# CliMA/ClimaOcean.jl

Measured on AMD Instinct MI355X. Metric: flux-kernel surface cells/s (update_state!: JRA55 interp + similarity-theory fluxes + net fluxes), higher is better.
Workload: dtype f64; 1 GPU; 1/4-degree LatitudeLongitudeGrid surface 1440x560 per job, JRA55 640x320 f32 atmosphere (4-snapshot window, clock advancing 20 min per step), SimilarityTheoryFluxes(:default) + Radiation, halo 7, ring 1; global_cells=806400, parallelism=latitude-slab x1, rows_per_rank=560, halo_backend=none, halo_rows=0, pipelined_interpolation=True, pipeline_mode=tail, step_loop=cf_time_steps (C)

## Files before the change

climaocean.jl_amd/coflux/abi.py:

```python
import ctypes as C
import os

import numpy as np

ABI_VERSION = 5
COMM_ID_BYTES = 128
PEER_HANDLE_BYTES = 64
HALO_NONE, HALO_RCCL, HALO_PEER = 0, 1, 2
FOLD_CENTER, FOLD_X_FACE, FOLD_Y_FACE = 0, 1, 2
SKIN_EXPLICIT, SKIN_SEMI_IMPLICIT, SKIN_LINEARISED = 0, 1, 2

SIMILARITY_LOGARITHMIC, SIMILARITY_COARE_LOGARITHMIC = 0, 1
STABILITY_EDSON2013, STABILITY_SHEBA, STABILITY_LARGE_YEAGER = 0, 1, 2
ROUGHNESS_CONSTANT, ROUGHNESS_CHARNOCK, ROUGHNESS_WIND_CHARNOCK = 0, 1, 2
SCALAR_ROUGHNESS_CONSTANT, SCALAR_ROUGHNESS_REYNOLDS = 0, 1
VISCOSITY_CONSTANT, VISCOSITY_TEMPERATURE_DEPENDENT = 0, 1
STOP_CONVERGENCE, STOP_FIXED = 0, 1
FORMULATION_SIMILARITY, FORMULATION_LARGE_YEAGER = 0, 1
VELOCITY_RELATIVE, VELOCITY_WIND = 0, 1
MASK_NONE, MASK_U8, MASK_BOTTOM_HEIGHT = 0, 1, 2
ALBEDO_CONSTANT, ALBEDO_LATITUDE_DEPENDENT = 0, 1
OPT_SOLVER, OPT_TRIP_HINTS, OPT_FUSED_NET, OPT_ICE_ORBIT_SHORTCUT, OPT_MERGED_PREFETCH = 0, 3, 6, 7, 9
OPT_INTERP_TILE_CAP, OPT_AO_CHUNK = 1, 4
OPT_INTERP_TILE_ROWS = 15
OPT_SOLVER_PATH, OPT_CERTIFIED_BUDGET, OPT_ICE_FREE_CELLS, OPT_LATENCY_LAYOUT, OPT_HALO_IN_SOLVER_LAUNCH = 10, 11, 12, 13, 14
OPT_LAND_ZEROS = 2
LAND_ZEROS_EVERY_LAUNCH, LAND_ZEROS_AUTO, LAND_ZEROS_NEVER = 0, 1, 2
ICE_FREE_ITERATE, ICE_FREE_ZERO = 0, 1
PIPELINE_WITHIN_CALL, PIPELINE_CONTINUING = 1, 2
AVERAGE_MAX_FIELDS = 16
DERIVED_MAX_SOURCES = 16
(TERM_FIELD, TERM_PRODUCT, TERM_CENTER_X, TERM_CENTER_Y, TERM_CENTER_X_SQUARE, TERM_CENTER_Y_SQUARE, TERM_KINETIC_ENERGY,
 TERM_EAST, TERM_NORTH) = range(9)
TERM_AT_CENTERS = 1
(BUDGET_HEAT_SHORTWAVE, BUDGET_HEAT_LONGWAVE_UP, BUDGET_HEAT_LONGWAVE_DOWN, BUDGET_HEAT_SENSIBLE, BUDGET_HEAT_LATENT,
 BUDGET_HEAT_ATMOSPHERE_OCEAN, BUDGET_HEAT_ICE_OCEAN, BUDGET_HEAT_FRAZIL, BUDGET_HEAT_NET, BUDGET_SALT_EVAPORATION,
 BUDGET_SALT_PRECIPITATION, BUDGET_SALT_ATMOSPHERE_OCEAN, BUDGET_SALT_ICE_OCEAN, BUDGET_SALT_LAND,
 BUDGET_SALT_NET) = range(15)
BUDGET_KINDS = 15
ATTACHED_AVERAGES_MAX = 4
INTEGRALS_MAX_ENTRIES, INTEGRALS_MAX_FIELDS = 32, 32
INTEGRAND_ONE, INTEGRAND_FIELD, INTEGRAND_PRODUCT, INTEGRAND_ABOVE = 0, 1, 2, 3
MONITOR_MAX_ENTRIES = 16
MONITOR_VALUE, MONITOR_ABS = 0, 1
CLIMATOLOGY_MAX_FIELDS, CLIMATOLOGY_MAX_BINS = 16, 32
CHECKPOINT_MAX_SECTIONS = 256
CHECKPOINT_DIRECT = 1
REGRID_MAX_FIELDS = 16
REGRID_MEAN, REGRID_SUM = 0, 1
SOLVER_PATH_EXACT, SOLVER_PATH_CERTIFIED = 0, 1
CERTIFIED_EXACT_FLAG = 0x100
SOLVER_TABLES, SOLVER_LIBM = 0, 1
STAGE_INTERPOLATE, STAGE_AO_FLUXES, STAGE_NET_FLUXES, STAGE_UPDATE_STATE = 0, 1, 2, 3

JRA55_VARIABLES = ("tas", "huss", "psl", "uas", "vas", "rlds", "rsds", "prra", "prsn")
JRA55_NVARS = len(JRA55_VARIABLES)

c_double_p = C.POINTER(C.c_double)
c_float_p = C.POINTER(C.c_float)
c_int32_p = C.POINTER(C.c_int32)


class Grid(C.Structure):
    _fields_ = [("nx", C.c_int32), ("ny", C.c_int32), ("hx", C.c_int32), ("hy", C.c_int32),
                ("ring", C.c_int32), ("reserved", C.c_int32)]


class Roughness(C.Structure):
    _fields_ = [("kind", C.c_int32), ("viscosity_kind", C.c_int32),
                ("constant_length", C.c_double), ("maximum_length", C.c_double),
                ("charnock", C.c_double), ("laminar", C.c_double),
                ("wind_a1", C.c_double), ("wind_a2", C.c_double), ("wind_umax", C.c_double),
                ("reynolds_A", C.c_double), ("reynolds_b", C.c_double),
                ("viscosity", C.c_double * 4)]


class Thermodynamics(C.Structure):
    _fields_ = [("gas_constant", C.c_double), ("dry_air_molar_mass", C.c_double),
                ("water_molar_mass", C.c_double), ("kappa_d", C.c_double),
                ("cp_v", C.c_double), ("cp_l", C.c_double), ("cp_i", C.c_double),
                ("LH_v0", C.c_double), ("LH_s0", C.c_double),
                ("T_0", C.c_double), ("T_triple", C.c_double), ("p_triple", C.c_double),
                ("T_freeze", C.c_double), ("T_icenuc", C.c_double), ("pow_icenuc", C.c_double)]


class Seawater(C.Structure):
    _fields_ = [("water_molar_mass", C.c_double),
                ("constituent_molar_mass", C.c_double * 4),
                ("constituent_mass_fraction", C.c_double * 4)]


class FluxParams(C.Structure):
    _fields_ = [("struct_size", C.c_int32), ("abi_version", C.c_int32),
                ("similarity_form", C.c_int32), ("stability_functions", C.c_int32),
                ("stop_kind", C.c_int32), ("maxiter", C.c_int32),
                ("velocity_difference", C.c_int32), ("mask_kind", C.c_int32),
                ("tolerance", C.c_double), ("von_karman", C.c_double),
                ("gustiness_parameter", C.c_double), ("minimum_gustiness", C.c_double),
                ("shear_gustiness_coefficient", C.c_double),
                ("similarity_profile_floor", C.c_double),
                ("momentum_roughness", Roughness), ("temperature_roughness", Roughness),
                ("water_vapor_roughness", Roughness),
                ("reference_height", C.c_double), ("boundary_layer_height", C.c_double),
                ("gravitational_acceleration", C.c_double),
                ("thermo", Thermodynamics), ("seawater", Seawater),
                ("ocean_reference_density", C.c_double), ("ocean_heat_capacity", C.c_double),
                ("ocean_freshwater_density", C.c_double),
                ("ocean_temperature_offset", C.c_double), ("ocean_minimum_salinity", C.c_double),
                ("ocean_surface_z", C.c_double),
                ("ocean_albedo_kind", C.c_int32), ("penetrating_shortwave", C.c_int32),
# ... 136 lines not shown
class BudgetDesc(C.Structure):
    _fields_ = [("struct_size", C.c_int32), ("n_terms", C.c_int32), ("terms", C.POINTER(BudgetTerm)),
                ("ocean", C.POINTER(OceanSurface)), ("exchange", C.POINTER(ExchangeFields)), ("fluxes", C.POINTER(InterfaceFluxes)),
                ("ice", C.POINTER(SeaIceFields)), ("frazil_heat", C.c_void_p), ("land_freshwater", C.c_void_p),
                ("weights", C.POINTER(InterpWeights)), ("max_workgroups", C.c_int32), ("reserved", C.c_int32)]


class IntegralEntry(C.Structure):
    _fields_ = [("kind", C.c_int32), ("region_bit", C.c_int32), ("a", C.c_void_p), ("b", C.c_void_p),
                ("threshold", C.c_double)]


class IntegralsDesc(C.Structure):
    _fields_ = [("struct_size", C.c_int32), ("n_entries", C.c_int32),
                ("area", C.c_void_p), ("mask", C.c_void_p), ("region", C.c_void_p),
                ("max_workgroups", C.c_int32), ("reserved", C.c_int32),
                ("entries", IntegralEntry * INTEGRALS_MAX_ENTRIES)]


class MonitorEntry(C.Structure):
    _fields_ = [("a", C.c_void_p), ("kind", C.c_int32), ("reserved", C.c_int32)]


class MonitorDesc(C.Structure):
    _fields_ = [("struct_size", C.c_int32), ("n_entries", C.c_int32), ("mask", C.c_void_p), ("first_cell", C.c_int64),
                ("max_workgroups", C.c_int32), ("reserved", C.c_int32), ("entries", MonitorEntry * MONITOR_MAX_ENTRIES)]


class MonitorValue(C.Structure):
    _fields_ = [("minimum", C.c_double), ("maximum", C.c_double), ("argmin", C.c_int64), ("argmax", C.c_int64),
                ("nan_count", C.c_int64), ("inf_count", C.c_int64), ("first_nonfinite", C.c_int64), ("hash", C.c_uint64)]


MONITOR_VALUE_DTYPE = np.dtype([("minimum", "<f8"), ("maximum", "<f8"), ("argmin", "<i8"), ("argmax", "<i8"), ("nan_count", "<i8"),
                                ("inf_count", "<i8"), ("first_nonfinite", "<i8"), ("hash", "<u8")])
assert MONITOR_VALUE_DTYPE.itemsize == C.sizeof(MonitorValue) == 64


class ClimatologyDesc(C.Structure):
    _fields_ = [("struct_size", C.c_int32), ("n_fields", C.c_int32), ("n_bins", C.c_int32), ("max_workgroups", C.c_int32),
                ("sources", C.c_void_p * CLIMATOLOGY_MAX_FIELDS), ("totals", C.c_void_p * CLIMATOLOGY_MAX_FIELDS),
                ("bins", C.c_void_p * CLIMATOLOGY_MAX_FIELDS), ("reserved", C.c_int32 * 2)]


class DatasetDesc(C.Structure):
    _fields_ = [("struct_size", C.c_int32), ("ns_x", C.c_int32), ("ns_y", C.c_int32), ("n_levels", C.c_int32),
                ("periodic_x", C.c_int32), ("max_sweeps", C.c_int32), ("sweeps_per_launch", C.c_int32), ("max_workgroups", C.c_int32),
                ("fill_value", C.c_double), ("period", C.c_double), ("times", C.c_void_p), ("weights", InterpWeights)]


class RegridDesc(C.Structure):
    _fields_ = [("struct_size", C.c_int32), ("mode", C.c_int32), ("n_rows", C.c_int64), ("nnz", C.c_int64),
                ("row_ptr", C.c_void_p), ("col", C.c_void_p), ("weight", C.c_void_p), ("mask", C.c_void_p),
                ("max_workgroups", C.c_int32), ("reserved", C.c_int32)]


class CheckpointDesc(C.Structure):
    _fields_ = [("struct_size", C.c_int32), ("flags", C.c_int32), ("max_workgroups", C.c_int32), ("reserved", C.c_int32)]


class PrefetchStats(C.Structure):
    _fields_ = [("struct_size", C.c_int32), ("pending", C.c_int32)] + [(n, C.c_uint64) for n in (
        "requests", "launched_aux", "launched_tail", "launched_merged", "launched_ice_tail", "launched_own",
        "consumed", "mismatched", "voided", "superseded", "discarded", "step_interpolations")]


EXPORTED_SYMBOLS = (
    "cf_version", "cf_default_flux_params", "cf_create", "cf_destroy", "cf_last_error",
    "cf_set_flux_params", "cf_set_stream", "cf_set_option", "cf_debug_eval", "cf_debug_chunk_plan", "cf_sync",
    "cf_device_alloc", "cf_device_free", "cf_h2d", "cf_d2h",
    "cf_interpolate_atmosphere_state", "cf_compute_atmosphere_ocean_fluxes",
    "cf_compute_net_ocean_fluxes", "cf_update_state", "cf_normalize_salinity_flux",
    "cf_default_sea_ice_params", "cf_set_sea_ice_formulation", "cf_compute_atmosphere_sea_ice_fluxes",
    "cf_compute_net_sea_ice_fluxes", "cf_update_state_sea_ice",
    "cf_time_stage", "cf_time_copy", "cf_profile_enable", "cf_profile_read",
    "cf_comm_unique_id", "cf_comm_init", "cf_comm_destroy", "cf_halo_exchange_rows",
    "cf_peer_halo_export", "cf_peer_halo_connect", "cf_halo_exchange_rows_peer", "cf_peer_halo_stats", "cf_fold_north_halo",
    "cf_time_steps", "cf_prefetch_atmosphere_state",
    "cf_default_sea_ice_albedo_params", "cf_set_sea_ice_albedo", "cf_compute_sea_ice_albedo",
    "cf_default_ice_ocean_params", "cf_compute_sea_ice_ocean_fluxes",
    "cf_interpolate_land_freshwater", "cf_set_land_freshwater", "cf_materialize_salinity_restoring",
    "cf_window_create", "cf_window_destroy", "cf_window_host_buffer", "cf_window_wait_slot", "cf_window_commit",
    "cf_window_upload", "cf_window_find", "cf_window_source",
    "cf_ensure_chunk_table", "cf_debug_chunk_table", "cf_debug_interp_grid", "cf_debug_land_zero_launches", "cf_solver_path", "cf_solver_iteration_path", "cf_solver_latency_layout", "cf_comm_count", "cf_build_stamp", "cf_discard_prefetched_atmosphere_state",
    "cf_debug_prefetch_stats",
    "cf_average_create", "cf_average_destroy", "cf_average_reset", "cf_average_collect", "cf_average_weight", "cf_attach_average",
    "cf_average_create_derived", "cf_average_create_budget", "cf_attach_average_slot",
    "cf_integrals_create", "cf_integrals_destroy", "cf_integrals_collect", "cf_integrals_count", "cf_integrals_read",
    "cf_integrals_reset", "cf_attach_integrals",
    "cf_monitor_create", "cf_monitor_destroy", "cf_monitor_collect", "cf_monitor_count", "cf_monitor_read", "cf_monitor_status",
    "cf_monitor_reset", "cf_attach_monitor",
    "cf_climatology_create", "cf_climatology_destroy", "cf_climatology_reset", "cf_climatology_collect", "cf_climatology_weights",
    "cf_climatology_extremes", "cf_calendar_bin", "cf_attach_climatology",
    "cf_dataset_create", "cf_dataset_destroy", "cf_dataset_stage", "cf_dataset_level", "cf_dataset_read_source", "cf_dataset_stage_info",
    "cf_dataset_time_index", "cf_dataset_evaluate", "cf_materialize_dataset_restoring", "cf_attach_restoring_dataset",
    "cf_regrid_create", "cf_regrid_destroy", "cf_regrid_apply",
    "cf_prepare_coupled_step", "cf_time_steps_coupled",
    "cf_checkpoint_create", "cf_checkpoint_destroy", "cf_checkpoint_add_array", "cf_checkpoint_add_average", "cf_checkpoint_add_climatology",
    "cf_checkpoint_add_integrals", "cf_checkpoint_add_monitor", "cf_checkpoint_set_host_blob", "cf_checkpoint_capture", "cf_checkpoint_wait",
    "cf_checkpoint_restore", "cf_checkpoint_verify", "cf_checkpoint_hash", "cf_checkpoint_host_blob",
)

PACKAGE_DIR = os.path.dirname(os.path.abspath(__file__))
LIB_PATH = os.environ.get("LIBCOFLUX") or os.path.join(os.path.dirname(PACKAGE_DIR), "csrc", "libcoflux.so")


class CofluxLibraryMissing(RuntimeError):
    pass


_lib = None


def source_stamp():
    import glob
    import hashlib
    csrc = os.path.join(os.path.dirname(os.path.dirname(os.path.abspath(__file__))), "csrc")
    names = sorted(os.path.basename(f) for ext in ("hip", "cpp", "hpp", "h") for f in glob.glob(os.path.join(csrc, "*." + ext)))
    header = os.path.join(csrc, "..", "..", "include", "coflux.h")
    if not names or not os.path.exists(header):
        return None
    h = hashlib.sha256()
    tool = os.path.join(csrc, "tools", "gcn_sched.py")
    for f in [header] + [os.path.join(csrc, n) for n in names] + ([tool] if os.path.exists(tool) else []):
        h.update(open(f, "rb").read())
    return h.hexdigest()[:16]


def load_library(path=None):
    global _lib
    if _lib is not None and path is None:
        return _lib
    p = path or LIB_PATH
    if not os.path.exists(p):
        raise CofluxLibraryMissing(
            f"{p} not found: build it with `python __graft_entry__.py build` "
            "(hipcc --offload-arch=gfx950). The HIP library is the only compute path.")
    lib = C.CDLL(p)
    vp = C.c_void_p
    lib.cf_version.restype = C.c_int
    lib.cf_build_stamp.restype = C.c_char_p
    want, have = source_stamp(), lib.cf_build_stamp().decode()
    if want is not None and have != want and os.environ.get("COFLUX_ALLOW_STALE_LIBRARY") != "1":
        raise CofluxLibraryMissing(
            f"{p} was built from other sources than this tree's (stamp {have}, tree {want}): rebuild it with "
            "`python __graft_entry__.py build` (COFLUX_ALLOW_STALE_LIBRARY=1 loads it anyway: A/B builds only)")
    lib.cf_default_flux_params.argtypes = [C.POINTER(FluxParams)]
    lib.cf_create.argtypes = [C.POINTER(vp), C.c_int, C.POINTER(Grid), C.POINTER(FluxParams)]
    lib.cf_destroy.argtypes = [vp]
    lib.cf_last_error.argtypes = [vp]
    lib.cf_last_error.restype = C.c_char_p
    lib.cf_set_flux_params.argtypes = [vp, C.POINTER(FluxParams)]
    lib.cf_set_stream.argtypes = [vp, vp]
    lib.cf_set_option.argtypes = [vp, C.c_int, C.c_int]
    lib.cf_solver_iteration_path.argtypes = [vp, C.POINTER(C.c_int)]
    lib.cf_solver_latency_layout.argtypes = [vp, C.POINTER(C.c_int)]
    lib.cf_peer_halo_stats.argtypes = [vp, C.POINTER(C.c_ulonglong), C.POINTER(C.c_ulonglong)]
    lib.cf_discard_prefetched_atmosphere_state.argtypes = [vp]
    lib.cf_debug_prefetch_stats.argtypes = [vp, C.POINTER(PrefetchStats)]
    lib.cf_comm_count.argtypes = [vp, C.POINTER(C.c_int), C.POINTER(C.c_int), C.POINTER(C.c_int)]
    lib.cf_debug_eval.argtypes = [vp, C.c_int, C.c_int, vp, vp]
    lib.cf_debug_chunk_plan.argtypes = [C.c_longlong, C.c_int, C.c_int, C.POINTER(C.c_int), C.c_int]
    lib.cf_sync.argtypes = [vp]
    lib.cf_device_alloc.argtypes = [vp, C.c_size_t]
    lib.cf_device_alloc.restype = vp
    lib.cf_device_free.argtypes = [vp, vp]
    lib.cf_h2d.argtypes = [vp, vp, vp, C.c_size_t]
    lib.cf_d2h.argtypes = [vp, vp, vp, C.c_size_t]
    lib.cf_interpolate_atmosphere_state.argtypes = [
        vp, C.POINTER(AtmosSource), C.POINTER(InterpWeights), C.POINTER(ExchangeFields)]
    lib.cf_compute_atmosphere_ocean_fluxes.argtypes = [
        vp, C.POINTER(OceanSurface), C.POINTER(ExchangeFields), C.POINTER(InterfaceFluxes)]
    lib.cf_compute_net_ocean_fluxes.argtypes = [
        vp, C.POINTER(OceanSurface), C.POINTER(ExchangeFields), C.POINTER(InterfaceFluxes),
        C.POINTER(SeaIceFields), C.POINTER(InterpWeights), C.POINTER(NetOceanFluxes)]
    lib.cf_update_state.argtypes = [
        vp, C.POINTER(AtmosSource), C.POINTER(InterpWeights), C.POINTER(OceanSurface),
        C.POINTER(ExchangeFields), C.POINTER(InterfaceFluxes), C.POINTER(SeaIceFields),
        C.POINTER(NetOceanFluxes)]
    lib.cf_normalize_salinity_flux.argtypes = [vp, vp, vp, vp, vp, vp]
    lib.cf_default_sea_ice_params.argtypes = [C.POINTER(SeaIceParams)]
    lib.cf_set_sea_ice_formulation.argtypes = [vp, C.POINTER(FluxParams), C.POINTER(SeaIceParams)]
    lib.cf_compute_atmosphere_sea_ice_fluxes.argtypes = [
        vp, C.POINTER(SeaIceState), C.POINTER(OceanSurface), C.POINTER(ExchangeFields), C.POINTER(InterfaceFluxes)]
    lib.cf_compute_net_sea_ice_fluxes.argtypes = [
        vp, C.POINTER(SeaIceState), C.POINTER(OceanSurface), C.POINTER(ExchangeFields), C.POINTER(InterfaceFluxes),
        vp, vp, C.POINTER(NetSeaIceFluxes)]
    lib.cf_update_state_sea_ice.argtypes = [
        vp, C.POINTER(AtmosSource), C.POINTER(InterpWeights), C.POINTER(OceanSurface), C.POINTER(ExchangeFields),
        C.POINTER(InterfaceFluxes), C.POINTER(SeaIceFields), C.POINTER(NetOceanFluxes), C.POINTER(SeaIceState),
        C.POINTER(InterfaceFluxes), vp, vp, C.POINTER(NetSeaIceFluxes)]
    lib.cf_time_stage.argtypes = [
        vp, C.c_int, C.c_int, C.POINTER(AtmosSource), C.POINTER(InterpWeights),
        C.POINTER(OceanSurface), C.POINTER(ExchangeFields), C.POINTER(InterfaceFluxes),
        C.POINTER(SeaIceFields), C.POINTER(NetOceanFluxes), C.POINTER(C.c_double)]
    lib.cf_time_copy.argtypes = [vp, vp, vp, C.c_size_t, C.c_int, C.POINTER(C.c_double)]
    lib.cf_profile_enable.argtypes = [vp, C.c_int]
    lib.cf_profile_read.argtypes = [vp, C.c_int, C.POINTER(C.c_double), C.POINTER(C.c_int)]
    lib.cf_comm_unique_id.argtypes = [vp]
    lib.cf_comm_init.argtypes = [vp, vp, C.c_int, C.c_int]
    lib.cf_comm_destroy.argtypes = [vp]
    lib.cf_halo_exchange_rows.argtypes = [vp, C.POINTER(vp), C.c_int, C.c_int]
    lib.cf_peer_halo_export.argtypes = [vp, C.c_int, C.c_int, vp]
    lib.cf_peer_halo_connect.argtypes = [vp, vp, vp, C.c_int, C.c_int]
    lib.cf_halo_exchange_rows_peer.argtypes = [vp, C.POINTER(vp), C.c_int, C.c_int]
    lib.cf_fold_north_halo.argtypes = [vp, C.POINTER(vp), C.POINTER(C.c_int), C.POINTER(C.c_double), C.c_int, C.c_int]
    lib.cf_time_steps.argtypes = [
        vp, C.c_int64, C.c_int, C.POINTER(RunSchedule), C.POINTER(AtmosSource), C.POINTER(InterpWeights),
        C.POINTER(InterfaceFluxes), C.POINTER(SeaIceFields), C.POINTER(NetOceanFluxes)]
    lib.cf_prepare_coupled_step.argtypes = [vp, C.POINTER(CoupledPrepare)]
    lib.cf_time_steps_coupled.argtypes = [
        vp, C.c_int64, C.c_int, C.POINTER(RunSchedule), C.POINTER(AtmosSource), C.POINTER(InterpWeights),
        C.POINTER(InterfaceFluxes), C.POINTER(SeaIceFields), C.POINTER(NetOceanFluxes), C.POINTER(CoupledStep)]
    lib.cf_prefetch_atmosphere_state.argtypes = [vp, C.POINTER(AtmosSource), C.POINTER(InterpWeights), C.POINTER(ExchangeFields)]
    lib.cf_ensure_chunk_table.argtypes = [vp, vp]
    lib.cf_debug_chunk_table.argtypes = [vp, C.POINTER(C.c_int), C.POINTER(C.c_int), C.c_int, C.POINTER(C.c_int), C.POINTER(C.c_int)]
    lib.cf_debug_interp_grid.argtypes = [vp, C.POINTER(C.c_int), C.POINTER(C.c_int)]
    lib.cf_debug_land_zero_launches.argtypes = [vp, C.POINTER(C.c_int)]
    lib.cf_solver_path.argtypes = [vp, C.POINTER(C.c_int), C.POINTER(C.c_int)]
    lib.cf_default_sea_ice_albedo_params.argtypes = [C.POINTER(SeaIceAlbedoParams)]
    lib.cf_set_sea_ice_albedo.argtypes = [vp, C.POINTER(SeaIceAlbedoParams)]
    lib.cf_compute_sea_ice_albedo.argtypes = [vp, C.POINTER(SeaIceAlbedoParams), vp, vp, vp, vp]
    lib.cf_default_ice_ocean_params.argtypes = [C.POINTER(IceOceanParams)]
    lib.cf_compute_sea_ice_ocean_fluxes.argtypes = [vp, C.POINTER(IceOceanParams), C.POINTER(OceanSurface), vp, vp, vp,
                                                    C.POINTER(IceOceanFluxes)]
    lib.cf_interpolate_land_freshwater.argtypes = [vp, C.POINTER(LandSource), C.POINTER(InterpWeights), vp]
    lib.cf_set_land_freshwater.argtypes = [vp, vp]
    lib.cf_materialize_salinity_restoring.argtypes = [vp, C.c_double, vp, C.POINTER(OceanSurface), vp]
    lib.cf_window_create.argtypes = [vp, C.c_int32, C.c_int32, C.c_int32, C.POINTER(vp)]
    lib.cf_window_destroy.argtypes = [vp]
    lib.cf_window_host_buffer.argtypes = [vp, C.c_int32, C.c_int32]
    lib.cf_window_host_buffer.restype = C.POINTER(C.c_float)
    lib.cf_window_wait_slot.argtypes = [vp, C.c_int32]
    lib.cf_window_commit.argtypes = [vp, C.c_int32, C.c_int64]
    lib.cf_window_upload.argtypes = [vp, C.c_int64, C.POINTER(vp)]
    lib.cf_window_find.argtypes = [vp, C.c_int64]
    lib.cf_window_source.argtypes = [vp, C.c_int64, C.c_int64, C.c_double, C.POINTER(AtmosSource)]
    lib.cf_average_create.argtypes = [vp, C.c_int, C.POINTER(vp), C.POINTER(vp), C.POINTER(vp)]
    lib.cf_average_destroy.argtypes = [vp]
    lib.cf_average_reset.argtypes = [vp]
    lib.cf_average_collect.argtypes = [vp, C.c_double]
    lib.cf_average_weight.argtypes = [vp, C.POINTER(C.c_double), C.POINTER(C.c_int64)]
    lib.cf_attach_average.argtypes = [vp, vp, C.c_int32, C.c_double]
    lib.cf_average_create_derived.argtypes = [vp, C.POINTER(AverageDesc), C.POINTER(vp)]
    lib.cf_average_create_budget.argtypes = [vp, C.POINTER(BudgetDesc), C.POINTER(vp)]
    lib.cf_attach_average_slot.argtypes = [vp, C.c_int32, vp, C.c_int32, C.c_double]
    for family, desc in (("integrals", IntegralsDesc), ("monitor", MonitorDesc)):
        for name, args in (("create", [vp, C.POINTER(desc), C.c_int32, C.POINTER(vp)]), ("destroy", [vp]), ("collect", [vp, C.c_double]),
                           ("count", [vp, C.POINTER(C.c_int64)]), ("read", [vp, C.c_int64, C.c_int64, vp, c_double_p]), ("reset", [vp])):
            getattr(lib, f"cf_{family}_{name}").argtypes = args
        getattr(lib, f"cf_attach_{family}").argtypes = [vp, vp, C.c_int32, C.c_double, C.c_double]
    lib.cf_monitor_status.argtypes = [vp, C.POINTER(C.c_int64), C.POINTER(C.c_uint32)]
    lib.cf_climatology_create.argtypes = [vp, C.POINTER(ClimatologyDesc), C.POINTER(vp)]
    lib.cf_climatology_destroy.argtypes = [vp]
    lib.cf_climatology_reset.argtypes = [vp]
    lib.cf_climatology_collect.argtypes = [vp, C.c_int32, C.c_double]
    lib.cf_climatology_weights.argtypes = [vp, c_double_p, C.POINTER(C.c_int64), c_double_p, C.POINTER(C.c_int64)]
    lib.cf_climatology_extremes.argtypes = [vp, C.c_int32, vp, vp, vp, vp]
    lib.cf_calendar_bin.argtypes = [c_double_p, c_int32_p, C.c_int32, C.c_double, c_int32_p]
    lib.cf_attach_climatology.argtypes = [vp, vp, C.c_int32, C.c_double, C.c_double, C.c_double, c_double_p, c_int32_p, C.c_int32]
    lib.cf_dataset_create.argtypes = [vp, C.POINTER(DatasetDesc), C.POINTER(vp)]
    lib.cf_dataset_destroy.argtypes = [vp]
    lib.cf_dataset_stage.argtypes = [vp, C.c_int32, vp]
    lib.cf_dataset_level.argtypes = [vp, C.c_int32, C.POINTER(vp)]
    lib.cf_dataset_read_source.argtypes = [vp, vp]
    lib.cf_dataset_stage_info.argtypes = [vp, C.c_int32, c_int32_p, C.POINTER(C.c_int64), C.POINTER(C.c_int64)]
    lib.cf_dataset_time_index.argtypes = [c_double_p, C.c_int32, C.c_double, C.c_double, c_int32_p, c_int32_p, c_double_p]
    lib.cf_dataset_evaluate.argtypes = [vp, C.c_double, vp]
    lib.cf_materialize_dataset_restoring.argtypes = [vp, C.c_double, vp, C.c_double, C.POINTER(OceanSurface), vp]
    lib.cf_attach_restoring_dataset.argtypes = [vp, vp, C.c_double, C.c_double]
    lib.cf_regrid_create.argtypes = [vp, C.POINTER(RegridDesc), C.POINTER(vp)]
    lib.cf_regrid_destroy.argtypes = [vp]
    lib.cf_regrid_apply.argtypes = [vp, C.c_int32, C.POINTER(vp), C.POINTER(vp), vp]
    lib.cf_checkpoint_create.argtypes = [vp, C.POINTER(CheckpointDesc), C.POINTER(vp)]
    lib.cf_checkpoint_destroy.argtypes = [vp]
    lib.cf_checkpoint_add_array.argtypes = [vp, C.c_char_p, vp, C.c_size_t]
    for kind in ("average", "climatology", "integrals", "monitor"):
        getattr(lib, "cf_checkpoint_add_" + kind).argtypes = [vp, C.c_char_p, vp]
    lib.cf_checkpoint_set_host_blob.argtypes = [vp, vp, C.c_size_t]
    lib.cf_checkpoint_capture.argtypes = [vp]
    lib.cf_checkpoint_wait.argtypes = [vp, C.POINTER(vp), C.POINTER(C.c_size_t)]
    lib.cf_checkpoint_restore.argtypes = [vp, vp, C.c_size_t]
    lib.cf_checkpoint_verify.argtypes = [vp, C.c_size_t]
    lib.cf_checkpoint_hash.argtypes = [vp, C.c_size_t, C.POINTER(C.c_uint64)]
    lib.cf_checkpoint_host_blob.argtypes = [vp, C.c_size_t, C.POINTER(vp), C.POINTER(C.c_size_t)]
    for name in EXPORTED_SYMBOLS:
        fn = getattr(lib, name)
        if name not in ("cf_last_error", "cf_device_alloc", "cf_window_host_buffer", "cf_build_stamp"):
            fn.restype = C.c_int
    if path is None:
        _lib = lib
    return lib
```

climaocean.jl_amd/coflux/runtime.py:

```python
import ctypes as C

import numpy as np
import torch

from . import abi

EXCHANGE_NAMES = ("u", "v", "T", "p", "q", "Qs", "Ql", "Mp")
FLUX_NAMES = ("sensible_heat", "latent_heat", "water_vapor", "x_momentum", "y_momentum", "temperature")
FLUX_OPTIONAL = ("friction_velocity", "temperature_scale", "humidity_scale")
NET_NAMES = ("u", "v", "T", "S", "shortwave_surface_flux", "upwelling_longwave",
             "downwelling_longwave", "downwelling_shortwave")
ICE_NAMES = ("concentration", "interface_heat", "salt_flux", "x_stress", "y_stress")


class CofluxError(RuntimeError):
    pass


def _ptr(t):
    return None if t is None else C.c_void_p(t.data_ptr())


def _is_field(t, ctx, dtype=torch.float64):
    return t.is_cuda and t.is_contiguous() and tuple(t.shape) == ctx.shape and dtype in (None, t.dtype)
# ... 191 lines not shown
    def set_land_freshwater(self, field):
        self._land = field
        self._check(self.lib.cf_set_land_freshwater(self._h, _ptr(field)), "cf_set_land_freshwater")

    def materialize_salinity_restoring(self, piston_velocity, target, ocean, out):
        o = self.ocean_struct(ocean)
        self._check(self.lib.cf_materialize_salinity_restoring(self._h, float(piston_velocity), _ptr(target), C.byref(o), _ptr(out)),
                    "cf_materialize_salinity_restoring")

    def compute_net_ocean_fluxes(self, ocean, atmos, fluxes, net, ice=None, weights=None):
        o, e, f = self.ocean_struct(ocean), self.exchange_struct(atmos), self.fluxes_struct(fluxes)
        i = self.ice_struct(ice)
        w = self.weights_struct(weights)
        n = self.net_struct(net)
        self._check(self.lib.cf_compute_net_ocean_fluxes(self._h, C.byref(o), C.byref(e), C.byref(f),
                                                         C.byref(i) if i is not None else None,
                                                         C.byref(w), C.byref(n)),
                    "cf_compute_net_ocean_fluxes")

    def update_state(self, src, weights, ocean, atmos, fluxes, net, ice=None, level1=0, level2=1,
                     time_fraction=0.0):
        s = self.source_struct(src, level1, level2, time_fraction)
        w = self.weights_struct(weights)
        o, e, f = self.ocean_struct(ocean), self.exchange_struct(atmos), self.fluxes_struct(fluxes)
        i = self.ice_struct(ice)
        n = self.net_struct(net)
        self._check(self.lib.cf_update_state(self._h, C.byref(s), C.byref(w), C.byref(o), C.byref(e),
                                             C.byref(f), C.byref(i) if i is not None else None, C.byref(n)),
                    "cf_update_state")

    def update_state_sea_ice(self, src, weights, ocean, atmos, fluxes, net, ice, ice_state, ai_fluxes, net_ice,
                             frazil_heat=None, interface_heat=None, level1=0, level2=1, time_fraction=0.0):
        s = self.source_struct(src, level1, level2, time_fraction)
        w = self.weights_struct(weights)
        o, e, f = self.ocean_struct(ocean), self.exchange_struct(atmos), self.fluxes_struct(fluxes)
        i = self.ice_struct(ice)
        n = self.net_struct(net)
        st = self._struct(abi.SeaIceState, ice_state, ("concentration", "thickness", "top_temperature", "u", "v", "albedo", "snow_thickness"))
        af = self.fluxes_struct(ai_fluxes)
        ni = self._struct(abi.NetSeaIceFluxes, net_ice, ("top_heat", "bottom_heat"))
        self._check(self.lib.cf_update_state_sea_ice(
            self._h, C.byref(s), C.byref(w), C.byref(o), C.byref(e), C.byref(f), C.byref(i) if i is not None else None,
            C.byref(n), C.byref(st), C.byref(af), frazil_heat.data_ptr() if frazil_heat is not None else None,
            interface_heat.data_ptr() if interface_heat is not None else None, C.byref(ni)), "cf_update_state_sea_ice")

    def time_stage(self, stage, launches, *, src=None, weights=None, ocean=None, atmos=None, fluxes=None,
                   net=None, ice=None, level1=0, level2=1, time_fraction=0.0):
        s = self.source_struct(src, level1, level2, time_fraction) if src is not None else abi.AtmosSource()
        w = self.weights_struct(weights)
        o, e, f = self.ocean_struct(ocean), self.exchange_struct(atmos), self.fluxes_struct(fluxes)
        i = self.ice_struct(ice)
        n = self.net_struct(net)
        ms = C.c_double()
        self._check(self.lib.cf_time_stage(self._h, stage, launches, C.byref(s), C.byref(w), C.byref(o),
                                           C.byref(e), C.byref(f), C.byref(i) if i is not None else None,
                                           C.byref(n), C.byref(ms)), "cf_time_stage")
        return ms.value

    def ensure_chunk_table(self, mask):
        self._check(self.lib.cf_ensure_chunk_table(self._h, _ptr(mask)), "cf_ensure_chunk_table")

    def debug_chunk_table(self):
        n, valid = C.c_int(), C.c_int()
        capacity = 1024
        while True:
            begins, counts = np.zeros(capacity, dtype=np.int32), np.zeros(capacity, dtype=np.int32)
            rc = self.lib.cf_debug_chunk_table(self._h, begins.ctypes.data_as(C.POINTER(C.c_int)),
                                               counts.ctypes.data_as(C.POINTER(C.c_int)), capacity, C.byref(n), C.byref(valid))
            if rc != 0 and n.value + 1 > capacity:
                capacity = n.value + 1
                continue
            self._check(rc, "cf_debug_chunk_table")
            return begins[:n.value + 1].copy(), counts[:n.value].copy(), bool(valid.value)

    def debug_interp_grid(self):
        rows, blocks = C.c_int(), C.c_int()
        self._check(self.lib.cf_debug_interp_grid(self._h, C.byref(rows), C.byref(blocks)), "cf_debug_interp_grid")
        return rows.value, blocks.value

    def debug_land_zero_launches(self):
        n = C.c_int()
        self._check(self.lib.cf_debug_land_zero_launches(self._h, C.byref(n)), "cf_debug_land_zero_launches")
        return n.value

    def solver_path(self):
        lean, fused = C.c_int(), C.c_int()
        self._check(self.lib.cf_solver_path(self._h, C.byref(lean), C.byref(fused)), "cf_solver_path")
        return bool(lean.value), fused.value

    def solver_iteration_path(self):
        path = C.c_int()
        self._check(self.lib.cf_solver_iteration_path(self._h, C.byref(path)), "cf_solver_iteration_path")
        return path.value

    def solver_latency_layout(self):
        layout = C.c_int()
        self._check(self.lib.cf_solver_latency_layout(self._h, C.byref(layout)), "cf_solver_latency_layout")
        return bool(layout.value)

    def time_copy(self, nbytes, launches=20):
        a = torch.empty(nbytes // 8, dtype=torch.float64, device=self.device)
        b = torch.empty_like(a)
        ms = C.c_double()
        self._check(self.lib.cf_time_copy(self._h, _ptr(b), _ptr(a), nbytes, launches, C.byref(ms)),
                    "cf_time_copy")
        return ms.value

    def normalize_salinity_flux(self, flux, mask, additional=None, area=None, mean_out=None):
        self._check(self.lib.cf_normalize_salinity_flux(self._h, _ptr(flux), _ptr(additional), _ptr(area), _ptr(mask),
                                                        _ptr(mean_out)), "cf_normalize_salinity_flux")

    def profile_enable(self, max_records):
        self._check(self.lib.cf_profile_enable(self._h, max_records), "cf_profile_enable")

    def profile_read(self, kernel):
        ms, n = C.c_double(), C.c_int()
        self._check(self.lib.cf_profile_read(self._h, kernel, C.byref(ms), C.byref(n)), "cf_profile_read")
        return ms.value, n.value

    def prefetch_atmosphere_state(self, src, weights, atmos_next, level1=0, level2=1, time_fraction=0.0):
        s = self.source_struct(src, level1, level2, time_fraction)
        w = self.weights_struct(weights)
        e = self.exchange_struct(atmos_next)
        self._check(self.lib.cf_prefetch_atmosphere_state(self._h, C.byref(s), C.byref(w), C.byref(e)),
                    "cf_prefetch_atmosphere_state")

    def discard_prefetched_atmosphere_state(self):
        self._check(self.lib.cf_discard_prefetched_atmosphere_state(self._h), "cf_discard_prefetched_atmosphere_state")

    def prefetch_stats(self):
        st = abi.PrefetchStats()
        st.struct_size = C.sizeof(abi.PrefetchStats)
        self._check(self.lib.cf_debug_prefetch_stats(self._h, C.byref(st)), "cf_debug_prefetch_stats")
        return {n: int(getattr(st, n)) for n, _ in abi.PrefetchStats._fields_ if n != "struct_size"}

    def make_schedule(self, ocean_states, atmos_sets, *, first_level=0, time_fraction=0.0, time_fraction_increment=0.0,
                      pipeline=False, halo_backend=abi.HALO_NONE, halo_rows=0, fold_north=False):
        sch = abi.RunSchedule()
        oc = (abi.OceanSurface * len(ocean_states))(*[self.ocean_struct(o) for o in ocean_states])
        at = (abi.ExchangeFields * len(atmos_sets))(*[self.exchange_struct(a) for a in atmos_sets])
        sch.struct_size = C.sizeof(abi.RunSchedule)
        sch.n_ocean_states, sch.ocean_states = len(ocean_states), oc
        sch.n_atmos_sets, sch.atmos, sch.pipeline = len(atmos_sets), at, int(pipeline)
        sch.first_level, sch.halo_backend, sch.halo_rows = first_level, halo_backend, halo_rows
        sch.fold_north = 1 if fold_north else 0
        sch.time_fraction, sch.time_fraction_increment = float(time_fraction), float(time_fraction_increment)
        sch._keep = (oc, at, ocean_states, atmos_sets)
        return sch

    def time_steps(self, first_step, nsteps, schedule, src, weights, fluxes, net, ice=None):
        s = self.source_struct(src, 0, 0, 0.0)
        w = self.weights_struct(weights)
        f, n, i = self.fluxes_struct(fluxes), self.net_struct(net), self.ice_struct(ice)
        self._check(self.lib.cf_time_steps(self._h, first_step, nsteps, C.byref(schedule), C.byref(s), C.byref(w),
                                           C.byref(f), C.byref(i) if i is not None else None, C.byref(n)),
                    "cf_time_steps")

    ICE_STATE_NAMES = ("concentration", "thickness", "top_temperature", "u", "v", "albedo", "snow_thickness")

    def _land_struct(self, friver, licalvf, level1=0, level2=0, time_fraction=0.0):
        s = abi.LandSource()
        if friver is not None:
            assert friver.dtype == torch.float32 and friver.is_cuda and friver.is_contiguous()
            s.friver = friver.data_ptr()
            s.licalvf = licalvf.data_ptr() if licalvf is not None else None
            s.n_levels, s.ns_y, s.ns_x = friver.shape
# ... 702 lines not shown
```

climaocean.jl_amd/csrc/coflux_abi.cpp:

```cpp
#include "coflux_ctx.hpp"

static thread_local std::string g_error;
static RcclApi g_rccl;

int cf_fail(cf_ctx* ctx, int code, const char* fmt, ...) {
    char buf[1024];
    va_list ap;
    va_start(ap, fmt);
    vsnprintf(buf, sizeof buf, fmt, ap);
    va_end(ap);
    g_error = buf;
    if (ctx) {
        std::lock_guard<std::mutex> lock(ctx->error_mutex);
        ctx->error = buf;
    }
    return code;
}

static int wait_for_halos(cf_ctx* ctx);

static bool roughness_ok(const cf_roughness& r, bool scalar) {
    if (scalar) {
        if (r.kind == CF_SCALAR_ROUGHNESS_CONSTANT) return r.constant_length > 0;
        if (r.kind == CF_SCALAR_ROUGHNESS_REYNOLDS) return r.maximum_length > 0 && r.reynolds_A > 0;
// ... 129 lines not shown
    C.b_q = q.reynolds_b;
    C.log_A_q = lg(q.reynolds_A);
    C.log_lm_q = lg(q.maximum_length);
    C.log_const_q = lg(q.constant_length);
    C.b_t = t.reynolds_b;
    C.log_A_t = lg(t.reynolds_A);
    C.log_lm_t = lg(t.maximum_length);
    C.log_const_t = lg(t.constant_length);
    C.maxiter = p.maxiter;
    C.fixed = p.stop_kind == CF_STOP_FIXED;
    C.m_kind = m.kind;
    C.q_kind = q.kind;
    C.t_kind = t.kind;
    C.same_scalar = std::memcmp(&t, &q, sizeof(cf_roughness)) == 0;
    const bool gusty = p.minimum_gustiness > 0;
    if (gusty && m.kind != CF_ROUGHNESS_CONSTANT && q.kind == CF_SCALAR_ROUGHNESS_REYNOLDS && C.same_scalar)
        C.specialization = SOLVER_OCEAN_LEAN;
    else if (gusty && m.kind == CF_ROUGHNESS_CONSTANT && q.kind == CF_SCALAR_ROUGHNESS_CONSTANT &&
             t.kind == CF_SCALAR_ROUGHNESS_CONSTANT)
        C.specialization = SOLVER_ICE;
    else
        C.specialization = SOLVER_GENERIC;
    if (p.flux_formulation == CF_FORMULATION_LARGE_YEAGER) {
        C.specialization = SOLVER_LY;
        C.ly_min_wind = p.ly_minimum_wind;
        C.ly_zeta_bound = p.ly_zeta_bound;
        C.ly_cd0 = p.ly_cd[0];
        C.ly_cd1 = p.ly_cd[1];
        C.ly_cd2 = p.ly_cd[2];
        C.ly_cd3 = p.ly_cd[3];
        C.ly_high_wind = p.ly_high_wind;
        C.ly_cd_high = p.ly_cd_high;
        C.ly_ce = p.ly_ce;
        C.ly_ch_s = p.ly_ch_stable;
        C.ly_ch_u = p.ly_ch_unstable;
        C.ly_lz = std::log(d.h_ref / 10.0);
    }
    C.inv_kappa = 1.0 / d.kappa;
    C.gust_c = d.beta_gust * d.beta_gust * d.beta_gust * d.h_bl / d.kappa;
    C.min_gust2 = d.min_gust * d.min_gust;
    C.x_scale = PSI_A * d.h_ref;
    C.two_inv_kappa = 2.0 / d.kappa;
    C.cert_u0 = 0.035;
    C.cert_two_inv_u0 = 2.0 / C.cert_u0;
    C.cert_chi0 = d.kappa / std::log(d.h_ref / 1e-4);
    C.cert_accept = 0x1p-23;
    C.cert_budget = 8e-7 / CERT_SAFETY;
    C.cert_max_evals = 10;
    return C;
}

static int ensure_chunk_table(cf_ctx* ctx, const void* mask) {
    const DevParams& d = ctx->dev;
    const void* key = d.mask_kind == CF_MASK_NONE ? nullptr : mask;
    if (ctx->chunk_valid && ctx->chunk_mask == key && ctx->chunk_mask_kind == d.mask_kind &&
        ctx->chunk_z_surface == d.z_surface)
        return CF_OK;
    const int ncells = (ctx->grid.nx + 2 * ctx->grid.ring) * (ctx->grid.ny + 2 * ctx->grid.ring);
    if (!ctx->d_chunk_sums) HIP_TRY(ctx, ctx->d_chunk_sums.create(sizeof(int) * chunk_sums_capacity(ncells)));
    if (!ctx->d_chunk_begins) HIP_TRY(ctx, ctx->d_chunk_begins.create(sizeof(int) * chunk_table_capacity(ncells)));
    if (!ctx->d_chunk_meta) HIP_TRY(ctx, ctx->d_chunk_meta.create(sizeof(int) * 4));
    int *const d_chunk_begins = ctx->d_chunk_begins.get(), *const d_chunk_meta = ctx->d_chunk_meta.get();
    int wet = 0, n = 0;
    const int plan = (ctx->launch.ao_chunk == 0 && ctx->merged_prefetch == 2 && !ctx->ice_ready) ? AO_PLAN_TAIL : ctx->launch.ao_chunk;
    HIP_TRY(ctx, build_chunk_table(ctx->stream, ctx->d_params.get(), ctx->grid, mask, ctx->launch.cu_count, plan,
                                   ctx->d_chunk_sums.get(), d_chunk_begins, d_chunk_meta, &wet, &n));
    {
        const size_t want = std::max(wet_list_capacity(ncells), (size_t)(n + 1) * wet_list_stride());
        if (want > ctx->wet.entries) {
            HIP_TRY(ctx, hipStreamSynchronize(ctx->stream));
            ctx->wet = cf_ctx::WetLists{};
            ctx->chunk_valid = false;
            cf_ctx::WetLists lists;
            HIP_TRY(ctx, lists.d_wet_pos.create(sizeof(uint32_t) * want));
            HIP_TRY(ctx, lists.d_lean_sorted.create(sizeof(uint32_t) * want));
            HIP_TRY(ctx, lists.d_lean_info.create(sizeof(int) * 4 * (size_t)chunk_table_capacity(ncells)));
            HIP_TRY(ctx, lists.d_trip.create(want));
            HIP_TRY(ctx, lists.d_trip_ice.create(want));
            lists.entries = want;
            ctx->wet = std::move(lists);
        }
    }
    if (n <= 0 || n + 1 > chunk_table_capacity(ncells)) return fail(ctx, CF_ERR_HIP, "chunk table of %d entries is invalid", n);
    ctx->chunk_mask = key;
    ctx->chunk_mask_kind = d.mask_kind;
    ctx->chunk_z_surface = d.z_surface;
    ctx->chunk_wet = wet;
    ctx->chunk_valid = true;
    ctx->launch.d_chunk_begins = d_chunk_begins;
    ctx->launch.n_chunks = n;
    {
        std::vector<int> begins((size_t)n + 1);
        HIP_TRY(ctx, hipMemcpyAsync(begins.data(), d_chunk_begins, sizeof(int) * begins.size(), hipMemcpyDeviceToHost, ctx->stream));
        HIP_TRY(ctx, hipStreamSynchronize(ctx->stream));
        const long wx = ctx->grid.nx + 2 * ctx->grid.ring, south_cells = (long)ctx->grid.ring * wx,
                   north_from = (long)(ctx->grid.ny - 1 + ctx->grid.ring) * wx;
        int cs = 0, cn = n;
        while (cs < n && begins[cs] < south_cells) ++cs;
        while (cn > 0 && begins[cn] > north_from) --cn;
        ctx->launch.chunk_south = cs;
        ctx->launch.chunk_north = cn;
    }
    int overflow = 0;
    const cf_ctx::WetLists& W = ctx->wet;
    HIP_TRY(ctx, build_wet_lists(ctx->stream, ctx->d_params.get(), ctx->grid, mask, n, d_chunk_begins, W.d_wet_pos.get(),
                                 W.d_trip.get(), d_chunk_meta, &overflow));
    ctx->launch.d_wet_pos = overflow ? nullptr : W.d_wet_pos.get();
    ctx->launch.d_lean_sorted = nullptr;
    ctx->launch.d_lean_info = nullptr;
    if (!overflow) HIP_TRY(ctx, build_lean_lists(ctx->stream, n, W.d_wet_pos.get(), d_chunk_begins, W.d_lean_sorted.get(), W.d_lean_info.get()));
    ctx->launch.d_lean_sorted = W.d_lean_sorted.get();
    ctx->launch.d_lean_info = W.d_lean_info.get();
    HIP_TRY(ctx, hipMemsetAsync(W.d_trip_ice.get(), 0, (size_t)n * wet_list_stride(), ctx->stream));
    ctx->launch.d_trip = ctx->trip_hints ? W.d_trip.get() : nullptr;
    if (std::getenv("COFLUX_DEBUG"))
        std::fprintf(stderr, "[coflux] chunk table: %d chunks of %d wet cells (%d CUs)\n", n, wet, ctx->launch.cu_count);
    return CF_OK;
}

static int install_params(cf_ctx* ctx, const cf_flux_params* params) {
    DevParams d;
    int rc = lower_params(ctx, params, &d);
    if (rc != CF_OK) return rc;
    if (ctx->tables_kind != d.stability) {
        std::vector<double> t = build_solver_tables(d.stability);
        if (hipSetDevice(ctx->device) != hipSuccess) return fail(ctx, CF_ERR_HIP, "hipSetDevice(%d) failed", ctx->device);
        if (!ctx->d_tables && ctx->d_tables.create(sizeof(double) * TABLE_DOUBLES) != hipSuccess)
            return fail(ctx, CF_ERR_HIP, "hipMalloc of the solver tables failed");
        if (hipMemcpy(ctx->d_tables.get(), t.data(), sizeof(double) * TABLE_DOUBLES, hipMemcpyHostToDevice) != hipSuccess)
            return fail(ctx, CF_ERR_HIP, "upload of the solver tables failed");
        ctx->tables_kind = d.stability;
        ctx->launch.d_tables = ctx->d_tables.get();
    }
    ctx->params = *params;
    ctx->dev = d;
    ctx->fast = loop_params(*params, d);
    ctx->fast.cert_budget = ctx->certified_budget / CERT_SAFETY;
    if (!ctx->d_params && ctx->d_params.create(sizeof(DevParams)) != hipSuccess)
        return fail(ctx, CF_ERR_HIP, "hipMalloc of the device parameter block failed");
    if (hipMemcpy(ctx->d_params.get(), &d, sizeof(DevParams), hipMemcpyHostToDevice) != hipSuccess)
        return fail(ctx, CF_ERR_HIP, "upload of the device parameter block failed");
    ctx->launch.d_params = ctx->d_params.get();
    ctx->chunk_valid = false;
    return CF_OK;
}

template <class Launch>
static int time_launches(cf_ctx* ctx, int launches, double* ms_per_launch, Launch launch) {
    HIP_TRY(ctx, hipSetDevice(ctx->device));
    cf::Event t0, t1;
    HIP_TRY(ctx, t0.create(hipEventDefault));
    HIP_TRY(ctx, t1.create(hipEventDefault));
    CHECK(launch());
    HIP_TRY(ctx, hipEventRecord(t0.get(), ctx->stream));
    for (int n = 0; n < launches; ++n) CHECK(launch());
    HIP_TRY(ctx, hipEventRecord(t1.get(), ctx->stream));
    HIP_TRY(ctx, hipEventSynchronize(t1.get()));
    float ms = 0.f;
    HIP_TRY(ctx, hipEventElapsedTime(&ms, t0.get(), t1.get()));
    *ms_per_launch = (double)ms / launches;
    return CF_OK;
}

void cf_peer_forget_local(const char* mailbox);

extern "C" {
// ... 162 lines not shown
int cf_set_option(cf_ctx* ctx, int option, int value) {
    if (!ctx) return fail(nullptr, CF_ERR_INVALID, "ctx is NULL");
    switch (option) {
        case CF_OPT_SOLVER:
            if (value != CF_SOLVER_TABLES && value != CF_SOLVER_LIBM) return fail(ctx, CF_ERR_INVALID, "unknown solver %d", value);
            ctx->launch.solver = value;
            return CF_OK;
        case CF_OPT_INTERP_TILE_CAP:
            if (!experiments_enabled()) return fail(ctx, CF_ERR_INVALID, "CF_OPT_INTERP_TILE_CAP is an experiment option: start the process with COFLUX_EXPERIMENTS=1");
            if (value != 0 && (value < 16 || value > 224)) return fail(ctx, CF_ERR_INVALID, "interp tile cap %d: 0 (LDS-free gather kernel) or 16…224", value);
            ctx->launch.interp_cap = value;
            return CF_OK;
        case CF_OPT_INTERP_TILE_ROWS:
            if (!experiments_enabled()) return fail(ctx, CF_ERR_INVALID, "CF_OPT_INTERP_TILE_ROWS is an experiment option: start the process with COFLUX_EXPERIMENTS=1");
            if (value != 0 && value != 1 && value != 2 && value != 4) return fail(ctx, CF_ERR_INVALID, "interp tile rows %d: 0 (automatic), 1, 2 or 4", value);
            ctx->launch.interp_rows = value;
            return CF_OK;
        case CF_OPT_TRIP_HINTS:
            if (value < 0 || value > 3) return fail(ctx, CF_ERR_INVALID, "trip hints %d: 0 (off), 1 (on), 2 (automatic), 3 (on, the lean kernel in quarter-chunk windows)", value);
            if (ctx->lean_hints && value != 1 && value != 3) ctx->chunk_valid = false;
            if (ctx->launch.lean_hints != (value == 1 ? 1 : (value == 3 ? 4 : 0))) ctx->chunk_valid = false;
            ctx->trip_hints = value != 0;
            ctx->lean_hints = value == 1 || value == 3;
            ctx->launch.d_trip = ctx->trip_hints ? ctx->wet.d_trip.get() : nullptr;
            ctx->launch.lean_hints = value == 1 ? 1 : (value == 3 ? 4 : 0);
            return CF_OK;
        case CF_OPT_FUSED_NET:
            if (value < 0 || value > 2) return fail(ctx, CF_ERR_INVALID, "fused net fluxes %d: 0 (never), 1 (when possible), 2 (automatic)", value);
            ctx->fused_net = value;
            return CF_OK;
        case CF_OPT_MERGED_PREFETCH:
            if (value < 0 || value > 2)
                return fail(ctx, CF_ERR_INVALID, "merged prefetch %d: 0 (auxiliary stream), 1 (in the face-stress launch), 2 (tail workgroups of the solver launch)", value);
            if ((ctx->merged_prefetch == 2) != (value == 2)) ctx->chunk_valid = false;
            ctx->merged_prefetch = value;
            return CF_OK;
        case CF_OPT_ICE_ORBIT_SHORTCUT:
            ctx->ice_orbit_shortcut = value != 0;
            ctx->ice_kernel.orbit_shortcut = value != 0 ? 1.0 : 0.0;
            return CF_OK;
        case CF_OPT_ICE_FREE_CELLS:
            if (value != CF_ICE_FREE_ITERATE && value != CF_ICE_FREE_ZERO) return fail(ctx, CF_ERR_INVALID, "ice-free cells %d: 0 (iterate) or 1 (zero)", value);
            ctx->ice_free_zero = value == CF_ICE_FREE_ZERO;
            ctx->ice_kernel.ice_free_zero = ctx->ice_free_zero ? 1.0 : 0.0;
            return CF_OK;
        case CF_OPT_SOLVER_PATH:
            if (value != CF_SOLVER_PATH_EXACT && value != CF_SOLVER_PATH_CERTIFIED) return fail(ctx, CF_ERR_INVALID, "solver path %d: 0 (exact) or 1 (certified)", value);
            ctx->launch.certified = value;
            return CF_OK;
        case CF_OPT_HALO_IN_SOLVER_LAUNCH:
            if (value < 0 || value > 1) return fail(ctx, CF_ERR_INVALID, "halo rows in the solver launch %d: 0 (the exchange kernel of its own) or 1", value);
            if (value && !ctx->d_halo_counters) {
                HIP_TRY(ctx, hipSetDevice(ctx->device));
                cf::DeviceBuffer<unsigned long long> counters;
                HIP_TRY(ctx, counters.create(4 * sizeof(unsigned long long)));
                HIP_TRY(ctx, hipMemset(counters.get(), 0, 4 * sizeof(unsigned long long)));
                ctx->d_halo_counters = std::move(counters);
            }
            ctx->halo_in_launch = value;
            return CF_OK;
        case CF_OPT_LATENCY_LAYOUT:
            if (value < 0 || value > 2) return fail(ctx, CF_ERR_INVALID, "latency layout %d: 0 (never), 1 (automatic), 2 (always)", value);
            ctx->launch.latency_layout = value;
            return CF_OK;
        case CF_OPT_CERTIFIED_BUDGET:
            if (value < 50 || value > 1000000) return fail(ctx, CF_ERR_INVALID, "certified budget %d: 50 … 1000000 (units of 1e-9)", value);
            ctx->certified_budget = value * 1e-9;
            ctx->fast.cert_budget = ctx->certified_budget / CERT_SAFETY;
            return CF_OK;
        case CF_OPT_AO_CHUNK:
            if (!experiments_enabled()) return fail(ctx, CF_ERR_INVALID, "CF_OPT_AO_CHUNK is an experiment option: start the process with COFLUX_EXPERIMENTS=1");
            if (value != 0 && value != 256 && value != 512 && value != 768 && value != 1024 && value != 1280)
                return fail(ctx, CF_ERR_INVALID, "solver chunk %d: wet cells per workgroup must be 0 (automatic), 256, 512, 768, 1024 or 1280 "
                            "(uniform size)", value);
            ctx->launch.ao_chunk = value;
            ctx->chunk_valid = false;
            return CF_OK;
        case CF_OPT_LAND_ZEROS:
            if (value < 0 || value > 2) return fail(ctx, CF_ERR_INVALID, "land zeros %d: 0 (every launch), 1 (automatic: the first step of a cf_time_steps call), 2 (never)", value);
            if (value == 2 && !experiments_enabled())
                return fail(ctx, CF_ERR_INVALID, "CF_OPT_LAND_ZEROS = 2 is an experiment value: start the process with COFLUX_EXPERIMENTS=1");
            ctx->land_zeros = value;
            return CF_OK;
        default: return fail(ctx, CF_ERR_INVALID, "unknown option %d", option);
    }
}

int cf_debug_eval(cf_ctx* ctx, int function, int n, const double* d_x, double* d_y) {
    if (!ctx || !d_x || !d_y || n < 0) return fail(ctx, CF_ERR_INVALID, "cf_debug_eval: bad arguments");
    HIP_TRY(ctx, hipSetDevice(ctx->device));
    HIP_TRY(ctx, launch_debug_eval(ctx->stream, ctx->launch, function, n, d_x, d_y));
    return CF_OK;
}

int cf_set_stream(cf_ctx* ctx, void* hip_stream) {
    if (!ctx) return fail(nullptr, CF_ERR_INVALID, "ctx is NULL");
    hipStream_t next = hip_stream == CF_STREAM_LEGACY ? nullptr
                       : (hip_stream ? (hipStream_t)hip_stream : ctx->own_stream.get());
    if (next != ctx->stream) {
        if (ctx->ahead.any_left_on_main()) {
            HIP_TRY(ctx, hipSetDevice(ctx->device));
            cf::Event ev;
            HIP_TRY(ctx, ev.create(hipEventDisableTiming));
            HIP_TRY(ctx, hipEventRecord(ev.get(), ctx->stream));
            HIP_TRY(ctx, hipStreamWaitEvent(next, ev.get(), 0));
        }
    }
    ctx->stream = next;
    return CF_OK;
}

int cf_sync(cf_ctx* ctx) {
    if (!ctx) return fail(nullptr, CF_ERR_INVALID, "ctx is NULL");
    HIP_TRY(ctx, hipSetDevice(ctx->device));
    if (int rc = wait_for_halos(ctx)) return rc;
    const AheadLedger::Work flush = ctx->ahead.leave_aux();
    CHECK(cf_ahead_perform(ctx, &flush));
    HIP_TRY(ctx, hipStreamSynchronize(ctx->stream));
    if (ctx->aux.stream) HIP_TRY(ctx, hipStreamSynchronize(ctx->aux.stream.get()));
    if (ctx->d_peer_status && ctx->peer_seq) {
        int st = 0;
        HIP_TRY(ctx, hipMemcpy(&st, ctx->d_peer_status.get(), sizeof st, hipMemcpyDeviceToHost));
        if (st) {
            HIP_TRY(ctx, hipMemset(ctx->d_peer_status.get(), 0, sizeof st));
            return fail(ctx, CF_ERR_COMM, "peer-direct halo exchange timed out waiting for the %s neighbour's rows",
                        st == 1 ? "south" : "north");
        }
    }
    if (!ctx->checkpoints.empty()) CHECK(checkpoint_settle_restores(ctx));
    return CF_OK;
}

void* cf_device_alloc(cf_ctx* ctx, size_t bytes) {
    if (!ctx) return nullptr;
    void* p = nullptr;
    hipSetDevice(ctx->device);
    hipError_t e = hipMalloc(&p, bytes);
    if (e != hipSuccess) {
        fail(ctx, CF_ERR_HIP, "hipMalloc(%zu): %s", bytes, hipGetErrorString(e));
        return nullptr;
    }
    return p;
}

int cf_device_free(cf_ctx* ctx, void* d_ptr) {
    if (!ctx) return fail(nullptr, CF_ERR_INVALID, "ctx is NULL");
    HIP_TRY(ctx, hipFree(d_ptr));
    return CF_OK;
}

int cf_h2d(cf_ctx* ctx, void* d_dst, const void* h_src, size_t bytes) {
    if (!ctx) return fail(nullptr, CF_ERR_INVALID, "ctx is NULL");
    HIP_TRY(ctx, hipMemcpyAsync(d_dst, h_src, bytes, hipMemcpyHostToDevice, ctx->stream));
    HIP_TRY(ctx, hipStreamSynchronize(ctx->stream));
    return CF_OK;
}

int cf_d2h(cf_ctx* ctx, void* h_dst, const void* d_src, size_t bytes) {
    if (!ctx) return fail(nullptr, CF_ERR_INVALID, "ctx is NULL");
    HIP_TRY(ctx, hipMemcpyAsync(h_dst, d_src, bytes, hipMemcpyDeviceToHost, ctx->stream));
    HIP_TRY(ctx, hipStreamSynchronize(ctx->stream));
    return CF_OK;
}

static int check_source(cf_ctx* ctx, const cf_atmos_source* s) {
    if (!s) return fail(ctx, CF_ERR_INVALID, "atmosphere source is NULL");
// ... 19 lines not shown
static int check_ocean(cf_ctx* ctx, const cf_ocean_surface* o) {
    if (!o || !o->T || !o->S || !o->u || !o->v) return fail(ctx, CF_ERR_INVALID, "ocean surface fields are NULL");
    if (ctx->dev.mask_kind != CF_MASK_NONE && !o->mask)
        return fail(ctx, CF_ERR_INVALID, "mask_kind = %d but ocean mask is NULL", ctx->dev.mask_kind);
    return CF_OK;
}
static int check_fluxes(cf_ctx* ctx, const cf_interface_fluxes* f) {
    if (!f || !f->sensible_heat || !f->latent_heat || !f->water_vapor || !f->x_momentum || !f->y_momentum || !f->temperature)
        return fail(ctx, CF_ERR_INVALID, "interface flux fields are NULL");
    return CF_OK;
}
static int check_net(cf_ctx* ctx, const cf_net_ocean_fluxes* n, const cf_interp_weights* w) {
    if (!n || !n->u || !n->v || !n->T || !n->S) return fail(ctx, CF_ERR_INVALID, "net ocean flux fields are NULL");
    if (ctx->dev.albedo_kind == CF_ALBEDO_LATITUDE_DEPENDENT && (!w || !w->latitude))
        return fail(ctx, CF_ERR_INVALID, "latitude-dependent albedo needs cf_interp_weights.latitude");
    return CF_OK;
}

static int wait_for_halos(cf_ctx* ctx) {
    if (ctx->comm_pending) {
        HIP_TRY(ctx, hipStreamWaitEvent(ctx->stream, ctx->comm_lane.ev_comm_done.get(), 0));
        ctx->comm_pending = false;
    }
    return CF_OK;
}

int cf_ensure_chunk_table(cf_ctx* ctx, const void* mask) {
    if (!ctx) return fail(nullptr, CF_ERR_INVALID, "ctx is NULL");
    HIP_TRY(ctx, hipSetDevice(ctx->device));
    return ensure_chunk_table(ctx, mask);
}

int cf_debug_chunk_table(cf_ctx* ctx, int* begins, int* wet_counts, int capacity, int* n_chunks, int* lists_valid) {
    if (!ctx || !n_chunks || !lists_valid) return fail(ctx, CF_ERR_INVALID, "cf_debug_chunk_table: bad arguments");
    *n_chunks = 0;
    *lists_valid = 0;
    if (!ctx->chunk_valid || !ctx->d_chunk_begins || ctx->launch.n_chunks <= 0)
        return fail(ctx, CF_ERR_INVALID, "cf_debug_chunk_table: no chunk table is valid (cf_ensure_chunk_table first)");
    const int n = ctx->launch.n_chunks;
    *n_chunks = n;
    *lists_valid = ctx->launch.d_wet_pos ? 1 : 0;
    if (!begins || !wet_counts || capacity < n + 1)
        return fail(ctx, CF_ERR_INVALID, "cf_debug_chunk_table: %d ints are too few for %d chunks", capacity, n);
    HIP_TRY(ctx, hipSetDevice(ctx->device));
    std::vector<int> info((size_t)4 * n, 0);
    HIP_TRY(ctx, hipMemcpyAsync(begins, ctx->d_chunk_begins.get(), sizeof(int) * ((size_t)n + 1), hipMemcpyDeviceToHost, ctx->stream));
    if (ctx->wet.d_lean_info)
        HIP_TRY(ctx, hipMemcpyAsync(info.data(), ctx->wet.d_lean_info.get(), sizeof(int) * info.size(), hipMemcpyDeviceToHost, ctx->stream));
    HIP_TRY(ctx, hipStreamSynchronize(ctx->stream));
    for (int c = 0; c < n; ++c) wet_counts[c] = info[(size_t)4 * c];
    return CF_OK;
}

int cf_debug_prefetch_stats(cf_ctx* ctx, cf_prefetch_stats* out) {
    if (!ctx || !out) return fail(ctx, CF_ERR_INVALID, "cf_debug_prefetch_stats: bad arguments");
    if (out->struct_size != (int32_t)sizeof(cf_prefetch_stats))
        return fail(ctx, CF_ERR_INVALID, "cf_prefetch_stats.struct_size = %d, library expects %zu", out->struct_size, sizeof(cf_prefetch_stats));
    *out = ctx->ahead.stats();
    out->struct_size = (int32_t)sizeof(cf_prefetch_stats);
    return CF_OK;
}

int cf_debug_land_zero_launches(cf_ctx* ctx, int* launches) {
    if (!ctx || !launches) return fail(ctx, CF_ERR_INVALID, "cf_debug_land_zero_launches: bad arguments");
    *launches = ctx->step_loop.zero_launches;
    return CF_OK;
}

int cf_debug_interp_grid(cf_ctx* ctx, int* rows, int* blocks) {
    if (!ctx || !rows || !blocks) return fail(ctx, CF_ERR_INVALID, "cf_debug_interp_grid: bad arguments");
    interpolate_grid(ctx->launch, ctx->grid, rows, blocks);
    return CF_OK;
}

static bool interp_tile_fits(const cf_ctx* ctx, size_t lds_bytes) {
    return ctx->launch.interp_cap > 0 && (size_t)4 * CF_JRA55_NVARS * (size_t)ctx->launch.interp_cap * sizeof(double) <= lds_bytes;
}

static bool net_fluxes_fused(const cf_ctx* ctx) {
    const bool lean = ctx->fast.specialization == SOLVER_OCEAN_LEAN && ctx->launch.solver == CF_SOLVER_TABLES;
    const bool fixed_trips = ctx->fast.specialization == SOLVER_LY && ctx->launch.solver == CF_SOLVER_TABLES;
    return (ctx->fused_net == 1 || (ctx->fused_net == 2 && (lean || fixed_trips))) && ctx->launch.solver == CF_SOLVER_TABLES &&
           ctx->dev.albedo_kind == CF_ALBEDO_CONSTANT;
}

int cf_solver_iteration_path(cf_ctx* ctx, int* path) {
    if (!ctx || !path) return fail(ctx, CF_ERR_INVALID, "cf_solver_iteration_path: bad arguments");
    const bool lean = ctx->fast.specialization == SOLVER_OCEAN_LEAN && ctx->launch.solver == CF_SOLVER_TABLES;
    *path = lean && lean_certified_applies(ctx->launch, ctx->fast) ? CF_SOLVER_PATH_CERTIFIED : CF_SOLVER_PATH_EXACT;
    return CF_OK;
}

int cf_solver_latency_layout(cf_ctx* ctx, int* layout) {
    if (!ctx || !layout) return fail(ctx, CF_ERR_INVALID, "cf_solver_latency_layout: bad arguments");
    const bool lean = ctx->fast.specialization == SOLVER_OCEAN_LEAN && ctx->launch.solver == CF_SOLVER_TABLES;
    *layout = lean && ctx->chunk_valid && lean_line_applies(ctx->launch, ctx->fast, ctx->dev.similarity_form == CF_SIMILARITY_COARE_LOGARITHMIC) ? 1 : 0;
    return CF_OK;
}

int cf_solver_path(cf_ctx* ctx, int* lean_kernel, int* fused_net) {
    if (!ctx || !lean_kernel || !fused_net) return fail(ctx, CF_ERR_INVALID, "cf_solver_path: bad arguments");
    *lean_kernel = ctx->fast.specialization == SOLVER_OCEAN_LEAN && ctx->launch.solver == CF_SOLVER_TABLES;
    *fused_net = net_fluxes_fused(ctx) ? 1 : 0;
    return CF_OK;
}

int cf_interpolate_atmosphere_state(cf_ctx* ctx, const cf_atmos_source* src, const cf_interp_weights* w,
                                    const cf_exchange_fields* out) {
    if (!ctx) return fail(nullptr, CF_ERR_INVALID, "ctx is NULL");
    HIP_TRY(ctx, hipSetDevice(ctx->device));
    CHECK(check_source(ctx, src));
    CHECK(check_weights(ctx, w));
    CHECK(check_exchange(ctx, out, true));
    HIP_TRY(ctx, launch_interpolate(ctx->stream, ctx->launch, ctx->grid, src, w, out));
    return CF_OK;
}

int cf_compute_atmosphere_ocean_fluxes(cf_ctx* ctx, const cf_ocean_surface* ocean, const cf_exchange_fields* atmos,
                                       const cf_interface_fluxes* out) {
    if (!ctx) return fail(nullptr, CF_ERR_INVALID, "ctx is NULL");
    HIP_TRY(ctx, hipSetDevice(ctx->device));
    CHECK(check_ocean(ctx, ocean));
    CHECK(check_exchange(ctx, atmos, false));
    CHECK(check_fluxes(ctx, out));
    CHECK(wait_for_halos(ctx));
    if (ctx->launch.solver == CF_SOLVER_LIBM && ctx->params.flux_formulation == CF_FORMULATION_LARGE_YEAGER)
        return fail(ctx, CF_ERR_INVALID, "CF_SOLVER_LIBM implements SimilarityTheoryFluxes only");
    CHECK(ensure_chunk_table(ctx, ocean->mask));
    HIP_TRY(ctx, launch_ao_fluxes(ctx->stream, ctx->launch, ctx->dev, ctx->fast, ctx->grid, ocean, atmos, out));
    return CF_OK;
}

int cf_compute_net_ocean_fluxes(cf_ctx* ctx, const cf_ocean_surface* ocean, const cf_exchange_fields* atmos,
                                const cf_interface_fluxes* fluxes, const cf_sea_ice_fields* ice,
                                const cf_interp_weights* w, const cf_net_ocean_fluxes* out) {
    if (!ctx) return fail(nullptr, CF_ERR_INVALID, "ctx is NULL");
    HIP_TRY(ctx, hipSetDevice(ctx->device));
    CHECK(check_ocean(ctx, ocean));
    CHECK(check_exchange(ctx, atmos, true));
    CHECK(check_fluxes(ctx, fluxes));
    CHECK(check_net(ctx, out, w));
    CHECK(wait_for_halos(ctx));
    HIP_TRY(ctx, launch_net_fluxes(ctx->stream, ctx->dev, ctx->grid, ocean, atmos, fluxes, ice, w, out, ctx->d_land_freshwater));
    return CF_OK;
}

static int update_state_impl(cf_ctx* ctx, const cf_atmos_source* src, const cf_interp_weights* w,
                             const cf_ocean_surface* ocean, const cf_exchange_fields* atmos,
                             const cf_interface_fluxes* fluxes, const cf_sea_ice_fields* ice, const cf_net_ocean_fluxes* net,
                             bool hold_tail_work, bool* stress_held, OceanRider* ocean_rider = nullptr) {
    if (!ctx) return fail(nullptr, CF_ERR_INVALID, "ctx is NULL");
    HIP_TRY(ctx, hipSetDevice(ctx->device));
    const cf_ctx::HaloRequest halo_request = std::exchange(ctx->halo_request, cf_ctx::HaloRequest{});
    CHECK(check_source(ctx, src));
    CHECK(check_weights(ctx, w));
    CHECK(check_ocean(ctx, ocean));
    CHECK(check_exchange(ctx, atmos, true));
    CHECK(check_fluxes(ctx, fluxes));
    CHECK(check_net(ctx, net, w));
    CHECK(ensure_chunk_table(ctx, ocean->mask));
    const bool rec = ctx->prof_count < ctx->prof_capacity;
    const cf::Event* ev = rec ? &ctx->prof_events[4 * (size_t)ctx->prof_count] : nullptr;
    if (rec) HIP_TRY(ctx, hipEventRecord(ev[0].get(), ctx->stream));
    const AheadLedger::Stepped stepped = ctx->ahead.step(atmos->u, *src, *w);
    CHECK(cf_ahead_perform(ctx, &stepped.work));
    const bool fuse = net_fluxes_fused(ctx);
    if (stepped.interpolate) HIP_TRY(ctx, launch_interpolate(ctx->stream, ctx->launch, ctx->grid, src, w, atmos));
    if (rec) HIP_TRY(ctx, hipEventRecord(ev[1].get(), ctx->stream));
    CHECK(wait_for_halos(ctx));
    const AheadLedger::Record* next = ctx->ahead.waiting_for_other_set(atmos->u);
    const bool tail_lean = ctx->launch.d_lean_info && ctx->fast.specialization == SOLVER_OCEAN_LEAN && ctx->launch.solver == CF_SOLVER_TABLES;
    const bool tail_ly = ctx->fast.specialization == SOLVER_LY && ctx->launch.solver == CF_SOLVER_TABLES;
    const bool tail = fuse && !hold_tail_work && ctx->merged_prefetch == 2 && next && interp_tile_fits(ctx, 40960) && (tail_lean || tail_ly);
    const bool ride = hold_tail_work && ocean_rider && fuse && tail_lean && !rec;
    HaloRider halo_rider{};
    const HaloRider* halo = nullptr;
    if (halo_request.valid) {
        if (tail && tail_lean && !ride && ctx->d_halo_counters && lean_halo_rides(ctx->launch, ctx->fast)) {
            HaloRider& H = halo_rider;
            H.M = ctx->peer;
            H.F = halo_request.F;
            H.counters = ctx->d_halo_counters.get();
            H.seq = ctx->peer_seq + 1;
            for (int dir = 0; dir < 2; ++dir) {
                const bool neighbour = (dir == 0 ? ctx->peer.south : ctx->peer.north) != nullptr;
                H.expect_sent[dir] = ctx->halo_expect_sent[dir] + (neighbour ? (unsigned long long)H.F.n : 0ull);
                H.expect_done[dir] = ctx->halo_expect_done[dir] + (neighbour ? (unsigned long long)H.F.n : 0ull);
            }
            H.status = ctx->d_peer_status.get();
            H.rows = halo_request.rows;
            H.blocks = 2 * H.F.n;
            H.chunk_south = ctx->launch.chunk_south;
            H.chunk_north = ctx->launch.chunk_north;
            H.wait_south = ctx->peer.south != nullptr;
            H.wait_north = ctx->peer.north != nullptr;
            halo = &halo_rider;
        } else {
            CHECK(cf_peer_halo_launch_now(ctx, &halo_request.F, halo_request.rows));
        }
    }
    const unsigned way = 1u | (fuse ? 2u : 0u) | (ride ? 4u : 0u) | ((unsigned)ctx->fast.specialization << 3);
    const bool knows = ctx->launch.solver == CF_SOLVER_TABLES;
    const bool keep_land = knows && (ctx->land_zeros == 2 || (ctx->land_zeros == 1 && ctx->step_loop.open && ctx->step_loop.last_way == way));
    LaunchCfg L = ctx->launch;
    L.keep_land = keep_land ? 1 : 0;
    if (ride) {
        HIP_TRY(ctx, make_ocean_rider(L, ctx->dev, ctx->fast, ctx->grid, ocean, atmos, fluxes, ice, net, ctx->d_land_freshwater,
                                      ocean_rider));
    } else if (tail) {
        int rows = 4, blocks = 1;
        interpolate_grid(L, ctx->grid, &rows, &blocks);
        if (tail_lean) {
            HIP_TRY(ctx, launch_ao_fluxes_lean(ctx->stream, L, ctx->dev, ctx->fast, ctx->grid, ocean, atmos, fluxes, ice, net,
                                               ctx->d_land_freshwater, &next->src, &next->w, &next->out, rows, blocks, halo));
            if (halo) {
                ctx->peer_seq = halo->seq;
                ++ctx->halo_in_launch_count;
                for (int dir = 0; dir < 2; ++dir) {
                    ctx->halo_expect_sent[dir] = halo->expect_sent[dir];
                    ctx->halo_expect_done[dir] = halo->expect_done[dir];
                }
            }
        } else
            HIP_TRY(ctx, launch_ly_fluxes_with_tail(ctx->stream, L, ctx->dev, ctx->fast, ctx->grid, ocean, atmos, fluxes, ice, net,
                                                    ctx->d_land_freshwater, &next->src, &next->w, &next->out, rows, blocks));
        ctx->ahead.leave_main(next, AheadLedger::TAIL);
    } else
    HIP_TRY(ctx, launch_ao_fluxes(ctx->stream, L, ctx->dev, ctx->fast, ctx->grid, ocean, atmos, fluxes,
                                  fuse ? ice : nullptr, fuse ? net : nullptr, ctx->d_land_freshwater));
    if (ctx->step_loop.open && !keep_land) ++ctx->step_loop.zero_launches;
    const bool merge = fuse && !hold_tail_work && ctx->merged_prefetch == 1 && next && interp_tile_fits(ctx, 65536);
    if (ctx->merged_prefetch == 0) {
        const AheadLedger::Work behind_solver = ctx->ahead.leave_aux();
        CHECK(cf_ahead_perform(ctx, &behind_solver));
    }
    if (rec) HIP_TRY(ctx, hipEventRecord(ev[2].get(), ctx->stream));
    if (merge) {
        HIP_TRY(ctx, launch_interpolate_and_stress(ctx->stream, ctx->launch, ctx->dev, ctx->grid, &next->src, &next->w, &next->out, ocean,
                                                   fluxes, ice, net));
        ctx->ahead.leave_main(next, AheadLedger::MERGED);
    } else if (fuse && hold_tail_work) {
        if (stress_held) *stress_held = true;
    } else if (fuse)
        HIP_TRY(ctx, launch_net_stress(ctx->stream, ctx->dev, ctx->grid, ocean, fluxes, ice, net, keep_land));
    else
        HIP_TRY(ctx, launch_net_fluxes(ctx->stream, ctx->dev, ctx->grid, ocean, atmos, fluxes, ice, w, net, ctx->d_land_freshwater));
    if (rec) {
        HIP_TRY(ctx, hipEventRecord(ev[3].get(), ctx->stream));
        ++ctx->prof_count;
    }
    next = ctx->ahead.waiting_for_other_set(atmos->u);
    if (!hold_tail_work && ctx->merged_prefetch != 0 && next) {
        HIP_TRY(ctx, launch_interpolate(ctx->stream, ctx->launch, ctx->grid, &next->src, &next->w, &next->out));
        ctx->ahead.leave_main(next, AheadLedger::OWN);
    }
    if (ctx->step_loop.open) ctx->step_loop.last_way = way;
    return CF_OK;
}

int cf_update_state(cf_ctx* ctx, const cf_atmos_source* src, const cf_interp_weights* w,
                    const cf_ocean_surface* ocean, const cf_exchange_fields* atmos,
                    const cf_interface_fluxes* fluxes, const cf_sea_ice_fields* ice, const cf_net_ocean_fluxes* net) {
    return update_state_impl(ctx, src, w, ocean, atmos, fluxes, ice, net, false, nullptr);
}

int cf_profile_enable(cf_ctx* ctx, int max_records) {
    if (!ctx || max_records < 0) return fail(ctx, CF_ERR_INVALID, "cf_profile_enable: bad arguments");
    HIP_TRY(ctx, hipSetDevice(ctx->device));
    std::vector<cf::Event> events(4 * (size_t)max_records);
    for (cf::Event& e : events) HIP_TRY(ctx, e.create(hipEventDefault));
    ctx->prof_events = std::move(events);
    ctx->prof_capacity = max_records;
    ctx->prof_count = 0;
    return CF_OK;
}

int cf_profile_read(cf_ctx* ctx, int kernel, double* avg_ms, int* records) {
    if (!ctx || !avg_ms || kernel < 0 || kernel > 2) return fail(ctx, CF_ERR_INVALID, "cf_profile_read: bad arguments");
    HIP_TRY(ctx, hipStreamSynchronize(ctx->stream));
    double sum = 0.0;
    for (int n = 0; n < ctx->prof_count; ++n) {
        float ms = 0.f;
        HIP_TRY(ctx, hipEventElapsedTime(&ms, ctx->prof_events[4 * (size_t)n + kernel].get(),
                                        ctx->prof_events[4 * (size_t)n + kernel + 1].get()));
        sum += ms;
    }
    *avg_ms = ctx->prof_count ? sum / ctx->prof_count : 0.0;
    if (records) *records = ctx->prof_count;
    return CF_OK;
}

static int run_stage(cf_ctx* ctx, int stage, const cf_atmos_source* src, const cf_interp_weights* w,
                     const cf_ocean_surface* ocean, const cf_exchange_fields* atmos, const cf_interface_fluxes* fluxes,
                     const cf_sea_ice_fields* ice, const cf_net_ocean_fluxes* net) {
    switch (stage) {
        case CF_STAGE_INTERPOLATE: return cf_interpolate_atmosphere_state(ctx, src, w, atmos);
        case CF_STAGE_AO_FLUXES: return cf_compute_atmosphere_ocean_fluxes(ctx, ocean, atmos, fluxes);
        case CF_STAGE_NET_FLUXES: return cf_compute_net_ocean_fluxes(ctx, ocean, atmos, fluxes, ice, w, net);
        case CF_STAGE_UPDATE_STATE: return cf_update_state(ctx, src, w, ocean, atmos, fluxes, ice, net);
        default: return fail(ctx, CF_ERR_INVALID, "unknown stage %d", stage);
    }
}

int cf_time_stage(cf_ctx* ctx, int stage, int launches, const cf_atmos_source* src, const cf_interp_weights* w,
                  const cf_ocean_surface* ocean, const cf_exchange_fields* atmos, const cf_interface_fluxes* fluxes,
                  const cf_sea_ice_fields* ice, const cf_net_ocean_fluxes* net, double* ms_per_launch) {
    if (!ctx || !ms_per_launch || launches <= 0) return fail(ctx, CF_ERR_INVALID, "cf_time_stage: bad arguments");
    return time_launches(ctx, launches, ms_per_launch, [&] { return run_stage(ctx, stage, src, w, ocean, atmos, fluxes, ice, net); });
}

int cf_time_copy(cf_ctx* ctx, void* d_dst, const void* d_src, size_t bytes, int launches, double* ms_per_launch) {
    if (!ctx || !ms_per_launch || launches <= 0 || !d_dst || !d_src)
        return fail(ctx, CF_ERR_INVALID, "cf_time_copy: bad arguments");
    return time_launches(ctx, launches, ms_per_launch, [&]() -> int {
        HIP_TRY(ctx, launch_copy(ctx->stream, d_dst, d_src, bytes));
        return CF_OK;
    });
}

static int load_rccl(cf_ctx* ctx) {
    if (g_rccl.handle) return CF_OK;
    const char* names[] = {"librccl.so", "librccl.so.1", "/opt/rocm/lib/librccl.so"};
    void* h = nullptr;
    for (const char* n : names)
        if ((h = dlopen(n, RTLD_NOW | RTLD_GLOBAL | RTLD_NOLOAD))) break;
    if (!h && dlsym(RTLD_DEFAULT, "ncclCommInitRank")) h = dlopen(nullptr, RTLD_NOW);
    if (!h)
        for (const char* n : names)
            if ((h = dlopen(n, RTLD_NOW | RTLD_GLOBAL))) break;
    if (!h) return fail(ctx, CF_ERR_COMM, "cannot dlopen librccl.so: %s", dlerror());
#define SYM(field, name)                                                     \
    g_rccl.field = (decltype(g_rccl.field))dlsym(h, name);                   \
    if (!g_rccl.field) return fail(ctx, CF_ERR_COMM, "librccl lacks %s", name);
    SYM(GetUniqueId, "ncclGetUniqueId");
    SYM(CommInitRank, "ncclCommInitRank");
    SYM(CommDestroy, "ncclCommDestroy");
    SYM(GroupStart, "ncclGroupStart");
    SYM(GroupEnd, "ncclGroupEnd");
    SYM(Send, "ncclSend");
// ... 514 lines not shown
```

climaocean.jl_amd/csrc/coflux_ctx.hpp:

```cpp
#pragma once
#include <dlfcn.h>
#include <hip/hip_runtime.h>
#include <rccl/rccl.h>

#include <algorithm>
#include <cmath>
#include <cstdarg>
#include <cstdint>
#include <cstdio>
#include <cstdlib>
#include <cstring>
#include <mutex>
#include <string>
#include <utility>
#include <variant>
#include <vector>

#include "../../include/coflux.h"
#include "coflux_checkpoint.hpp"
#include "coflux_checkpoint_image.hpp"
#include "coflux_collect.hpp"
#include "coflux_dataset_rules.hpp"
#include "coflux_fast.hpp"
#include "coflux_kernel_types.hpp"
#include "coflux_kernels.h"
#include "coflux_owned.hpp"
#include "coflux_request_ahead.hpp"
#include "coflux_tables.h"

using namespace coflux;

#ifndef CF_LAND_ZEROS_DEFAULT
#define CF_LAND_ZEROS_DEFAULT 1
#endif
static_assert(CF_LAND_ZEROS_DEFAULT == 0 || CF_LAND_ZEROS_DEFAULT == 1, "the experiment value is not a default");

struct RcclApi {
    void* handle = nullptr;
    ncclResult_t (*GetUniqueId)(ncclUniqueId*) = nullptr;
    ncclResult_t (*CommInitRank)(ncclComm_t*, int, ncclUniqueId, int) = nullptr;
    ncclResult_t (*CommDestroy)(ncclComm_t) = nullptr;
    ncclResult_t (*GroupStart)() = nullptr;
    ncclResult_t (*GroupEnd)() = nullptr;
    ncclResult_t (*Send)(const void*, size_t, ncclDataType_t, int, ncclComm_t, hipStream_t) = nullptr;
    ncclResult_t (*Recv)(void*, size_t, ncclDataType_t, int, ncclComm_t, hipStream_t) = nullptr;
    const char* (*GetErrorString)(ncclResult_t) = nullptr;
    ncclResult_t (*AllReduce)(const void*, void*, size_t, ncclDataType_t, ncclRedOp_t, ncclComm_t, hipStream_t) = nullptr;
    ncclResult_t (*CommCount)(const ncclComm_t, int*) = nullptr;
    ncclResult_t (*CommUserRank)(const ncclComm_t, int*) = nullptr;
    ncclResult_t (*CommCuDevice)(const ncclComm_t, int*) = nullptr;
};

struct cf_child;
struct Attachment {
    cf_child* handle = nullptr;
    StepSchedule when;
    double step_weight = 0.0;
    bool collects(int64_t step) const { return handle && when.due(step); }
};

struct SectionPlan {
    uint32_t section;
    uint64_t offset;
    cfck::Entry& entry;
    uint64_t& device_bytes;
    std::vector<unsigned char>& tail;
    std::vector<CheckpointSegment>& segments;
};

struct cf_child {
    cf_ctx* ctx = nullptr;
    int device = 0;
    virtual ~cf_child() = default;
    virtual int admit(const Attachment& , const char* , int64_t , int ) const { return CF_OK; }
    virtual int collect_step(const Attachment& , int64_t ) { return CF_OK; }
    virtual uint32_t section_kind() const { return cfck::KINDS; }
    virtual void plan_section(const SectionPlan&, const int64_t* ) const {}
    virtual uint64_t section_room() const { return 0; }
    virtual int check_entry(const cfck::Entry&, const char* ) const { return CF_OK; }
    virtual void load_tail(const std::vector<unsigned char>&, int64_t ) {}
};

struct cf_ctx {
    int device = 0;
    GridDesc grid{};
    cf_flux_params params{};
    DevParams dev{};
    cf::Stream own_stream;
    hipStream_t stream = nullptr;
    LoopParams fast{};
    cf::DeviceBuffer<DevParams> d_params;
    LaunchCfg launch = [] {
        LaunchCfg L{};
        L.solver = CF_SOLVER_TABLES;
        L.interp_cap = 128;
        L.cu_count = 256;
        return L;
    }();
    struct WetLists {
        cf::DeviceBuffer<uint8_t> d_trip;
        cf::DeviceBuffer<uint32_t> d_wet_pos;
        cf::DeviceBuffer<uint32_t> d_lean_sorted;
        cf::DeviceBuffer<int> d_lean_info;
        cf::DeviceBuffer<uint8_t> d_trip_ice;
        size_t entries = 0;
    } wet;
    bool trip_hints = true;
    bool lean_hints = false;
    int merged_prefetch = 0;
    double certified_budget = 8e-7;
    int fused_net = 2;
    cf::DeviceBuffer<int> d_chunk_sums, d_chunk_begins, d_chunk_meta;
    const void* chunk_mask = nullptr;
    int chunk_mask_kind = -1;
    double chunk_z_surface = 0.0;
    int chunk_wet = 0;
    bool chunk_valid = false;
    cf::DeviceBuffer<double> d_reduce;
    bool ice_ready = false;
    cf_flux_params ice_params{};
    cf_sea_ice_params ice_props{};
    DevParams ice_dev{};
    LoopParams ice_loop{};
    IceParams ice_kernel{};
    bool ice_orbit_shortcut = true;
    bool ice_free_zero = false;
    const double* d_land_freshwater = nullptr;
    bool ice_albedo_ccsm3 = false;
    cf_sea_ice_albedo_params ice_albedo{};
    cf::DeviceBuffer<double> d_ice_albedo;
    cf::DeviceBuffer<double> d_ice_tables;
    cf::DeviceBuffer<DevParams> d_ice_params;
    struct CommLane {
        cf::Stream stream;
        cf::Event ev_main_idle, ev_comm_done;
    } comm_lane;
    bool comm_pending = false;
    cf::DeviceBuffer<double> d_tables;
    int tables_kind = -1;
    std::string error;
    std::mutex error_mutex;
    struct AuxLane {
        cf::Stream stream;
        cf::Event ev_gate;
        cf::Event done[2];
    } aux;
    AheadLedger ahead;
    PeerMailbox peer{};
    cf::DeviceBuffer<char> peer_mine;
    cf::IpcMapping peer_south_map, peer_north_map;
    int peer_max_fields = 0, peer_max_rows = 0;
    bool peer_connected = false;
    unsigned long long peer_seq = 0;
    cf::DeviceBuffer<int> d_peer_status;
    int halo_in_launch = 0;
    unsigned long long halo_in_launch_count = 0;
    cf::DeviceBuffer<unsigned long long> d_halo_counters;
    unsigned long long halo_expect_sent[2] = {0, 0}, halo_expect_done[2] = {0, 0};
    struct HaloRequest {
        bool valid = false;
        PeerFields F{};
        int rows = 0;
    } halo_request;
    int land_zeros = CF_LAND_ZEROS_DEFAULT;
    struct StepLoop {
        bool open = false;
        unsigned last_way = 0;
        int zero_launches = 0;
    } step_loop;
    ncclComm_t comm = nullptr;
    int rank = 0, nranks = 1;
    std::vector<cf::Event> prof_events;
    int prof_capacity = 0, prof_count = 0;
    std::vector<cf_child*> children;
    std::vector<struct cf_checkpoint*> checkpoints;
    enum { AT_CLIMATOLOGY = CF_ATTACHED_AVERAGES_MAX, AT_INTEGRALS, AT_MONITOR, AT_COUNT };
    Attachment attached[AT_COUNT];
    Attachment restoring_dataset;
};

struct LandZeroScope {
    cf_ctx* ctx;
    explicit LandZeroScope(cf_ctx* c) : ctx(c) {
        ctx->step_loop = cf_ctx::StepLoop{};
        ctx->step_loop.open = true;
    }
    ~LandZeroScope() {
        ctx->step_loop.open = false;
        ctx->step_loop.last_way = 0;
    }
    LandZeroScope(const LandZeroScope&) = delete;
    LandZeroScope& operator=(const LandZeroScope&) = delete;
};

struct HaloRequestScope {
    cf_ctx* ctx;
    explicit HaloRequestScope(cf_ctx* c) : ctx(c) { ctx->halo_request = cf_ctx::HaloRequest{}; }
    ~HaloRequestScope() { ctx->halo_request = cf_ctx::HaloRequest{}; }
    HaloRequestScope(const HaloRequestScope&) = delete;
    HaloRequestScope& operator=(const HaloRequestScope&) = delete;
};

struct PlainAverageArgs {
    int nfields;
    AverageFields fields;
};
struct cf_average : cf_child {
    std::variant<PlainAverageArgs, DerivedArgs, BudgetArgs> args;
    RunningWeight weight;
    int collect(double w);
    int collect_step(const Attachment& at, int64_t) override { return collect(at.when.stride * at.step_weight); }
    uint32_t section_kind() const override { return cfck::KIND_AVERAGE; }
    void plan_section(const SectionPlan& P, const int64_t*) const override {
        P.entry.bytes = RunningWeight::BYTES;
        P.tail.resize(RunningWeight::BYTES);
        weight.put(P.tail.data());
    }
    void load_tail(const std::vector<unsigned char>& tail, int64_t) override { weight.get(tail.data()); }
};

struct cf_climatology : cf_child {
    int n_fields = 0, n_bins = 0, max_blocks = 0;
    const double* src[CF_CLIMATOLOGY_MAX_FIELDS] = {};
    double* total[CF_CLIMATOLOGY_MAX_FIELDS] = {};
    double* bins[CF_CLIMATOLOGY_MAX_FIELDS] = {};
    RunningWeight weight;
    RunningWeight bin_weight[CF_CLIMATOLOGY_MAX_BINS];
    std::vector<double> edges;
    std::vector<int32_t> bin_of_interval;
    int collect(int32_t bin, double w);
    int admit(const Attachment& at, const char* fn, int64_t first_step, int nsteps) const override;
    int collect_step(const Attachment& at, int64_t step) override;
    uint32_t section_kind() const override { return cfck::KIND_CLIMATOLOGY; }
    void plan_section(const SectionPlan& P, const int64_t*) const override {
        P.entry.n_entries = (uint32_t)n_bins;
        P.entry.bytes = RunningWeight::BYTES + 16 * (uint64_t)n_bins;
        P.tail.resize((size_t)P.entry.bytes);
        put_binned_weights(P.tail.data(), weight, bin_weight, n_bins);
    }
    int check_entry(const cfck::Entry& E, const char* fn) const override;
    void load_tail(const std::vector<unsigned char>& tail, int64_t) override { get_binned_weights(tail.data(), &weight, bin_weight, n_bins); }
};

struct cf_dataset : cf_child {
    int ns_x = 0, ns_y = 0, n_levels = 0, max_sweeps = -1, sweeps_per_launch = 0, max_blocks = 0;
    bool periodic_x = false;
    double fill_value = 0.0, period = 0.0;
    std::vector<double> times;
    cf_interp_weights weights{};
    cf::DeviceBuffer<double> d_plane[2];
    cf::DeviceBuffer<float> d_upload;
    cf::DeviceBuffer<double> d_levels;
    cf::PinnedBuffer<float> h_upload[2];
    cf::Event uploaded[2];
    int upload_slot = 0, current = 0;
    int last_level = -1;
    struct Staged {
        bool done = false;
        int32_t sweeps = 0;
        int64_t filled = 0, defaulted = 0;
    } staged[CF_DATASET_MAX_LEVELS];
    size_t parent() const { return (size_t)ctx->grid.sj * (size_t)(ctx->grid.ny + 2 * ctx->grid.hy); }
    double* level(int l) const { return d_levels.get() + parent() * (size_t)l; }
    int first_unstaged() const {
        for (int l = 0; l < n_levels; ++l)
            if (!staged[l].done) return l;
        return -1;
    }
};
struct DatasetTarget {
    const double* level1;
    const double* level2;
    double fraction;
// ... 75 lines not shown
```

climaocean.jl_amd/csrc/coflux_kernels.h:

```cpp
#pragma once
#include <hip/hip_runtime.h>

#include <cstdlib>

#include "coflux_device.hpp"

namespace coflux {

inline bool experiments_enabled() {
    static const bool enabled = [] {
        const char* e = std::getenv("COFLUX_EXPERIMENTS");
        return e != nullptr && e[0] == '1';
    }();
    return enabled;
}

struct LoopParams;
struct IceParams;
struct HaloRider;

struct LaunchCfg {
    int solver;
    int interp_cap;
    int interp_rows;
    int ao_chunk;
    int cu_count;
    const double* d_tables;
    const DevParams* d_params;
    uint8_t* d_trip;
    const int* d_chunk_begins;
    int n_chunks;
    int chunk_south, chunk_north;
    const uint32_t* d_wet_pos;
    uint32_t* d_lean_sorted;
    const int* d_lean_info;
    int lean_hints;
    int certified;
    int latency_layout;
    int keep_land;
};

bool lean_line_applies(const LaunchCfg& L, const LoopParams& C, bool coare);

bool lean_certified_applies(const LaunchCfg& L, const LoopParams& C);

hipError_t launch_interpolate(hipStream_t st, const LaunchCfg& L, const GridDesc& G, const cf_atmos_source* s,
                              const cf_interp_weights* w, const cf_exchange_fields* e);
hipError_t launch_ao_fluxes(hipStream_t st, const LaunchCfg& L, const DevParams& P, const LoopParams& C,
                            const GridDesc& G, const cf_ocean_surface* o, const cf_exchange_fields* e,
                            const cf_interface_fluxes* f, const cf_sea_ice_fields* ice = nullptr,
                            const cf_net_ocean_fluxes* net = nullptr, const double* land = nullptr);
hipError_t launch_net_stress(hipStream_t st, const DevParams& P, const GridDesc& G, const cf_ocean_surface* o,
                             const cf_interface_fluxes* f, const cf_sea_ice_fields* ice, const cf_net_ocean_fluxes* n,
                             bool keep_land = false);
hipError_t build_wet_lists(hipStream_t st, const DevParams* d_params, const GridDesc& G, const void* mask, int nchunks,
                           const int* d_begins, uint32_t* d_wet_pos, uint8_t* d_trip, int* d_scratch, int* overflow_out);
hipError_t build_lean_lists(hipStream_t st, int nchunks, const uint32_t* d_wet_pos, const int* d_begins, uint32_t* d_sorted, int* d_info);
hipError_t launch_ly_fluxes_with_tail(hipStream_t st, const LaunchCfg& L, const DevParams& P, const LoopParams& C, const GridDesc& G,
                                      const cf_ocean_surface* o, const cf_exchange_fields* e, const cf_interface_fluxes* f,
                                      const cf_sea_ice_fields* ice, const cf_net_ocean_fluxes* net, const double* land,
                                      const cf_atmos_source* next_src, const cf_interp_weights* w, const cf_exchange_fields* next_out,
                                      int tail_rows, int tail_blocks);
hipError_t launch_ao_fluxes_lean(hipStream_t st, const LaunchCfg& L, const DevParams& P, const LoopParams& C, const GridDesc& G,
                                 const cf_ocean_surface* o, const cf_exchange_fields* e, const cf_interface_fluxes* f,
                                 const cf_sea_ice_fields* ice = nullptr, const cf_net_ocean_fluxes* net = nullptr, const double* land = nullptr,
                                 const cf_atmos_source* next_src = nullptr, const cf_interp_weights* w = nullptr,
                                 const cf_exchange_fields* next_out = nullptr, int tail_rows = 0, int tail_blocks = 0,
                                 const HaloRider* halo = nullptr);
bool lean_halo_rides(const LaunchCfg& L, const LoopParams& C);
size_t wet_list_capacity(int ncells);
int wet_list_stride();
hipError_t launch_ao_fluxes_libm(hipStream_t st, const DevParams& P, const GridDesc& G, const cf_ocean_surface* o,
                                 const cf_exchange_fields* e, const cf_interface_fluxes* f);
hipError_t launch_net_fluxes(hipStream_t st, const DevParams& P, const GridDesc& G, const cf_ocean_surface* o,
                             const cf_exchange_fields* e, const cf_interface_fluxes* f, const cf_sea_ice_fields* ice,
                             const cf_interp_weights* w, const cf_net_ocean_fluxes* n, const double* land = nullptr);
hipError_t launch_interpolate_land(hipStream_t st, const GridDesc& G, const cf_land_source* s, const cf_interp_weights* w, double* out);
hipError_t launch_salinity_restoring(hipStream_t st, const DevParams& P, const GridDesc& G, const void* mask, double vp,
                                     const double* target, const double* S, double* out);
void interpolate_grid(const LaunchCfg& L, const GridDesc& G, int* rows_out, int* blocks_out);
hipError_t launch_interpolate_and_stress(hipStream_t st, const LaunchCfg& L, const DevParams& P, const GridDesc& G,
                                         const cf_atmos_source* s, const cf_interp_weights* w, const cf_exchange_fields* e,
                                         const cf_ocean_surface* o, const cf_interface_fluxes* f, const cf_sea_ice_fields* ice,
                                         const cf_net_ocean_fluxes* n);
hipError_t launch_interpolate_background(hipStream_t st, const GridDesc& G, const cf_atmos_source* s,
                                         const cf_interp_weights* w, const cf_exchange_fields* e);
struct OceanRider {
    alignas(16) unsigned char args[1536];
    int n_chunks = 0;
    bool coare = false, valid = false;
};
hipError_t make_ocean_rider(const LaunchCfg& L, const DevParams& P, const LoopParams& C, const GridDesc& G, const cf_ocean_surface* o,
                            const cf_exchange_fields* e, const cf_interface_fluxes* f, const cf_sea_ice_fields* ice,
                            const cf_net_ocean_fluxes* net, const double* land, OceanRider* out);
struct AiTail {
    const OceanRider* ocean = nullptr;
    const cf_atmos_source* next_src = nullptr;
    const cf_interp_weights* w = nullptr;
    const cf_exchange_fields* next_out = nullptr;
    int interp_rows = 0, interp_blocks = 0;
    const DevParams* d_ocean_params = nullptr;
    const cf_ocean_surface* stress_ocean = nullptr;
    const cf_interface_fluxes* stress_fluxes = nullptr;
    const cf_sea_ice_fields* stress_ice = nullptr;
    const cf_net_ocean_fluxes* stress_net = nullptr;
};
hipError_t launch_ai_fluxes(hipStream_t st, const LaunchCfg& L, const DevParams& P, const LoopParams& C, const IceParams& I,
                            const GridDesc& G, const cf_sea_ice_state* ice, const cf_ocean_surface* o,
                            const cf_exchange_fields* e, const cf_interface_fluxes* f, const double* d_tables,
                            const DevParams* d_params, uint8_t* d_trip, const AiTail* tail = nullptr, const NetIceOut* net_ice = nullptr);
constexpr int AO_PLAN_TAIL = -2;
hipError_t build_chunk_table(hipStream_t st, const DevParams* d_params, const GridDesc& G, const void* mask, int cu_count,
                             int wet_per_chunk, int* d_sums, int* d_begins, int* d_meta, int* wet_per_chunk_out,
                             int* nchunks_out);
int chunk_table_capacity(int ncells);
int chunk_sums_capacity(int ncells);
hipError_t launch_net_sea_ice_fluxes(hipStream_t st, const DevParams& P, const GridDesc& G, const void* mask,
                                     const cf_sea_ice_state* ice, double albedo, double emissivity, double eps_sigma,
                                     double T_offset, const cf_exchange_fields* e, const cf_interface_fluxes* f,
                                     const double* frazil, const double* interface_heat, const cf_net_sea_ice_fluxes* out);
hipError_t launch_sea_ice_albedo(hipStream_t st, const cf_sea_ice_albedo_params& A, const GridDesc& G, const double* hi,
                                 const double* hs, const double* Ts, double* out);
// ... 158 lines not shown
```

climaocean.jl_amd/csrc/coflux_lean_kernel.hpp:

```cpp
#pragma once
#include <hip/hip_runtime.h>

#include "coflux_halo_device.hpp"
#include "coflux_interp_tiles.hpp"
#include "coflux_lean.hpp"
#include "coflux_certified.hpp"
#include "coflux_solver_shared.hpp"

namespace coflux {

constexpr int LEAN_WAVES = 3;

struct LeanArgs {
    LoopParams L;
    GridDesc G;
    OceanIn O;
    Exchange E;
    FluxOut F;
    const double* g_tab;
    const DevParams* g_params;
    uint32_t* sorted;
    const int* info;
    const int* chunk_begins;
    double z_surface;
    long long mask_kind;
    double T_offset;
    unsigned long long wx_reciprocal;
    long long sort_enabled;
    IceIn I;
    NetOut N;
    SourceDesc S;
    WeightDesc Wt;
    Exchange E_next;
    long long n_chunks;
    long long tail_blocks, tail_rows, tail_cap;
    long long tail_pos;
    HaloRider H;
    long long keep_land;
};
typedef const LeanArgs __attribute__((address_space(4)))* LeanArgsPtr;

hipError_t launch_ao_lean_line(hipStream_t st, bool coare, bool fuse, bool tail, bool halo, int blocks, const LeanArgs& A);

__device__ __forceinline__ LeanArgsPtr opaque(LeanArgsPtr p) {
    asm volatile("" : "+s"(p));
    return p;
}

__device__ __forceinline__ unsigned lean_mix(unsigned idx) { return (idx * 0x9e3779b1u) ^ ((idx * 0x85ebca6bu) >> 15); }
__device__ __forceinline__ unsigned lean_sum(unsigned idx) { return idx * 0xc2b2ae35u + 0x27d4eb2fu; }

constexpr int LEAN_LIST_OFFSET = TABLE_BYTES;
constexpr int LEAN_OFFSET_BITS = 24;
constexpr unsigned LEAN_OFFSET_MASK = (1u << LEAN_OFFSET_BITS) - 1u;
static_assert((long)AO_CHUNK * AO_WET_COST < (1L << LEAN_OFFSET_BITS), "a chunk's range must fit the offset bits");
template <int BLOCK>
struct LeanGeom {
    static_assert(BLOCK == AO_BLOCK, "one workgroup geometry: 256 threads, three workgroups per CU (the 768-thread one-per-CU geometry of rounds 2-5 measured 3 % slower and was retired in round 6)");
    static constexpr int CHUNK = AO_CHUNK;
    static constexpr int WAVES = BLOCK / 64;
    static constexpr int HIST_OFFSET = LEAN_LIST_OFFSET + CHUNK * 4;
    static constexpr int CURSOR_OFFSET = HIST_OFFSET + AO_BINS * 4;
    static constexpr int COUNTERS_OFFSET = CURSOR_OFFSET + AO_BINS * 4;
    static constexpr int WAVEHASH_OFFSET = COUNTERS_OFFSET + 16;
    static constexpr int PARAMS_OFFSET = WAVEHASH_OFFSET + WAVES * 8;
    static constexpr int LDS_BYTES = PARAMS_OFFSET + (int)sizeof(DevParams);
    static_assert(PARAMS_OFFSET % 16 == 0 && LEAN_LIST_OFFSET % 1024 == 0 && (CHUNK * 4) % 1024 == 0, "LDS-DMA pieces");
};
static_assert(LeanGeom<AO_BLOCK>::LDS_BYTES <= 53760, "three narrow lean solver workgroups must fit the CU's 160 KB of LDS");

template <bool FUSE>
__device__ __forceinline__ void lean_zero_cell(const LoopParams& L, double T_offset, const GridDesc& G, LeanArgsPtr K, size_t k, int i, int j) {
    CellFluxes Z{};
    Z.Ts_ocean = -T_offset;
    Z.iterations = L.fixed ? L.maxiter : 0;
    const FluxOut F = kread(&K->F);
    store_fluxes(F, k, Z);
    if constexpr (FUSE) {
        if (i >= 0 && i < G.nx && j >= 0 && j < G.ny) {
            const NetOut N = kread(&K->N);
            store_net_cell(N, k, NetCell{});
        }
    }
}

template <bool COARE, bool FUSE, bool TAIL = false, bool CERT = false, bool LINE = false, bool HALO = false>
__device__ __forceinline__ void ao_lean_body(LeanArgsPtr K_in, int chunk_in) {
    constexpr int BLOCK = AO_BLOCK;
    using Geo = LeanGeom<BLOCK>;
    constexpr int CHUNK = Geo::CHUNK;
    LeanArgsPtr K = opaque(K_in);
    int chunk = chunk_in;
    bool wait_south = false, wait_north = false;
    if constexpr (HALO) {
        static_assert(TAIL && !CERT, "the halo riders belong to the stepping loop's exact-path launch");
        const int nh = K->H.blocks;
        if (chunk < nh) {
            extern __shared__ __attribute__((aligned(16))) char smem_h[];
            const int nf = K->H.F.n, dir = chunk / nf, f = chunk - dir * nf;
            const PeerMailbox M = kread(&K->H.M);
            const GridDesc Gh = kread(&K->G);
            peer_halo_rider(M, K->H.F.ptr[f], f, dir, K->H.rows, K->H.seq, K->H.counters, K->H.expect_sent[dir], K->H.status, Gh, BLOCK,
                            reinterpret_cast<int*>(smem_h));
            return;
        }
        chunk -= nh;
    }
    if constexpr (TAIL) {
        static_assert(BLOCK == 64 * IT_WAVES, "a tail workgroup is an interpolation workgroup");
        const int nb = (int)K->tail_blocks, ipos = (int)K->tail_pos;
        if (chunk >= ipos && chunk < ipos + nb) {
            const SourceDesc S = kread(&K->S);
            const WeightDesc Wt = kread(&K->Wt);
            const GridDesc Gt = kread(&K->G);
            const Exchange En = kread(&K->E_next);
            const int b = chunk - ipos, cap = (int)K->tail_cap, rows = (int)K->tail_rows;
            if (rows == 4) interpolate_tiles<4>(S, Wt, Gt, En, cap, b, nb);
            else if (rows == 2) interpolate_tiles<2>(S, Wt, Gt, En, cap, b, nb);
            else interpolate_tiles<1>(S, Wt, Gt, En, cap, b, nb);
            return;
        }
        if (chunk >= ipos) chunk -= nb;
    }
    if constexpr (HALO) {
        const int cs = K->H.chunk_south, cn = K->H.chunk_north, nc = (int)K->n_chunks;
        if (K->H.blocks > 0) {
            if (cs <= cn) {
                const int inner = cn - cs;
                chunk = chunk < inner ? cs + chunk : (chunk - inner < cs ? chunk - inner : cn + (chunk - inner - cs));
            }
            wait_south = K->H.wait_south != 0 && chunk < cs;
            wait_north = K->H.wait_north != 0 && chunk >= cn && chunk < nc;
        }
    }
    const LoopParams L = kread(&K->L);
    const GridDesc G = kread(&K->G);
    const double* __restrict__ g_tab = K->g_tab;
    const DevParams* __restrict__ g_params = K->g_params;
    const void* mask = K->O.mask;
    extern __shared__ __attribute__((aligned(16))) char smem[];
    double* tab = reinterpret_cast<double*>(smem);
    unsigned* list = reinterpret_cast<unsigned*>(smem + LEAN_LIST_OFFSET);
    int* hist = reinterpret_cast<int*>(smem + Geo::HIST_OFFSET);
    int* cursor = reinterpret_cast<int*>(smem + Geo::CURSOR_OFFSET);
    int* counters = reinterpret_cast<int*>(smem + Geo::COUNTERS_OFFSET);
    unsigned* wavehash = reinterpret_cast<unsigned*>(smem + Geo::WAVEHASH_OFFSET);
    DevParams* lp = reinterpret_cast<DevParams*>(smem + Geo::PARAMS_OFFSET);
    const int tid = threadIdx.x, lane = tid & 63, wave = tid >> 6;
    const int wx = G.nx + 2 * G.ring;
    const unsigned wx_rcp = (unsigned)K->wx_reciprocal;
    const bool use_static = K->sorted != nullptr;
    static_assert(sizeof(DevParams) % 16 == 0 && sizeof(DevParams) <= 1024, "the parameter block is one LDS-DMA piece");
    if (tid < (int)(sizeof(DevParams) / 16))
        __builtin_amdgcn_global_load_lds((const __attribute__((address_space(1))) void*)(reinterpret_cast<const char*>(g_params) + lane * 16),
                                         (__attribute__((address_space(3))) void*)(smem + Geo::PARAMS_OFFSET), 16, 0, 0);
    static_assert(TABLE_BYTES % 1024 == 0, "the table stage copies whole 1 KB pieces");
    {
        const char* gb = reinterpret_cast<const char*>(g_tab);
        constexpr int PIECES = TABLE_BYTES / 1024, WAVES = Geo::WAVES;
#pragma unroll
        for (int r = 0; r < (PIECES + WAVES - 1) / WAVES; ++r) {
            const int c = wave + r * WAVES;
            if (c < PIECES)
                __builtin_amdgcn_global_load_lds((const __attribute__((address_space(1))) void*)(gb + c * 1024 + lane * 16),
                                                 (__attribute__((address_space(3))) void*)(smem + c * 1024), 16, 0, 0);
        }
    }
    if (use_static) {
        const char* gl = reinterpret_cast<const char*>(K->sorted + (size_t)chunk * CHUNK);
        constexpr int PIECES = CHUNK * 4 / 1024, WAVES = Geo::WAVES;
#pragma unroll
        for (int r = 0; r < (PIECES + WAVES - 1) / WAVES; ++r) {
            const int c = wave + r * WAVES;
            if (c < PIECES)
                __builtin_amdgcn_global_load_lds((const __attribute__((address_space(1))) void*)(gl + c * 1024 + lane * 16),
                                                 (__attribute__((address_space(3))) void*)(smem + LEAN_LIST_OFFSET + c * 1024), 16, 0, 0);
        }
    }
    constexpr int LAND_UNROLL = 8;
    typedef const __attribute__((address_space(1))) unsigned* GlobalWords;
    unsigned raw_lo[LAND_UNROLL], raw_hi[LAND_UNROLL], raw_shift = 0;
    const __attribute__((address_space(4))) int* cb = (const __attribute__((address_space(4))) int*)K->chunk_begins;
    const int range_begin = cb[chunk], range_end = cb[chunk + 1];
    int listed = 0;
    unsigned want_x = 0, want_y = 0;
    if (use_static) {
        const __attribute__((address_space(4))) int* ci = (const __attribute__((address_space(4))) int*)K->info;
        listed = ci[chunk * 4];
        want_x = (unsigned)ci[chunk * 4 + 1];
        want_y = (unsigned)ci[chunk * 4 + 2];
    }
    const int mask_kind = (mask == nullptr) ? CF_MASK_NONE : (int)K->mask_kind;
    const double z_surface = K->z_surface;
    const double T_offset = K->T_offset;
    const bool keep_land = K->keep_land != 0;
    const bool sorting = !CERT && use_static && K->sort_enabled != 0;
    const int sort_windows = (int)K->sort_enabled;
    float inv_window = 0.f;
    auto lean_bin = [&](int q, int trips) -> int {
        if (sort_windows <= 1) return AO_BINS - 1 - trip_bin(trips);
        const int w = min((int)(((float)q + 0.5f) * inv_window), sort_windows - 1);
        const int bpw = AO_BINS / sort_windows, lo = bpw >= 16 ? 5 : 8;
        return w * bpw + (bpw - 1 - min(max(trips - lo, 0), bpw - 1));
    };
    {
        const unsigned long long mbase = mask_kind == CF_MASK_NONE ? (unsigned long long)g_tab : (unsigned long long)mask;
        const unsigned stride = mask_kind == CF_MASK_NONE ? 0u : (mask_kind == CF_MASK_U8 ? 1u : 8u);
        const unsigned hi_step = mask_kind == CF_MASK_BOTTOM_HEIGHT ? 4u : 0u;
#pragma unroll
        for (int n = 0; n < LAND_UNROLL; ++n) {
            const int ic = min(range_begin + tid + n * BLOCK, range_end - 1);
            const int jj = row_of(ic, wx, wx_rcp);
            const unsigned long long a = mbase + (unsigned long long)cell_index(G, ic - jj * wx - G.ring, jj - G.ring) * stride;
            raw_shift |= ((unsigned)a & 3u) << (2 * n);
            raw_lo[n] = *(GlobalWords)(a & ~3ull);
            raw_hi[n] = *(GlobalWords)((a & ~3ull) + hi_step);
        }
    }
    if (tid < 4) counters[tid] = 0;
    if (tid < AO_BINS) hist[tid] = 0;
    if constexpr (CERT) {
        if (tid < 2 * AO_BINS) hist[tid] = -1;
    }
    __builtin_amdgcn_s_waitcnt(0x0f70);
#pragma unroll
    for (int n = 0; n < LAND_UNROLL; ++n) asm volatile("" : "+v"(raw_lo[n]), "+v"(raw_hi[n]));
    unsigned hx = 0, hy = 0, land = 0;
#pragma unroll
    for (int n = 0; n < LAND_UNROLL; ++n) {
        const int idx = range_begin + tid + n * BLOCK;
        const bool w = mask_kind == CF_MASK_NONE ? true
                       : mask_kind == CF_MASK_U8 ? ((raw_lo[n] >> (8 * ((raw_shift >> (2 * n)) & 3u))) & 0xffu) != 0
                                                 : !(z_surface <= __hiloint2double((int)raw_hi[n], (int)raw_lo[n]));
        if (idx < range_end) {
            if (w) {
                hx ^= lean_mix((unsigned)idx);
                hy += lean_sum((unsigned)idx);
            } else {
                land |= 1u << n;
            }
        }
    }
    for (int idx = range_begin + tid + LAND_UNROLL * BLOCK; idx < range_end; idx += BLOCK) {
        const int jj = row_of(idx, wx, wx_rcp);
        const size_t k = cell_index(G, idx - jj * wx - G.ring, jj - G.ring);
        const bool w = mask_kind == CF_MASK_NONE ? true
                       : mask_kind == CF_MASK_U8 ? ((const uint8_t*)mask)[k] != 0 : !(z_surface <= ((const double*)mask)[k]);
        if (w) {
            hx ^= lean_mix((unsigned)idx);
            hy += lean_sum((unsigned)idx);
        } else if (!keep_land) {
            lean_zero_cell<FUSE>(L, T_offset, G, opaque(K), k, idx - jj * wx - G.ring, jj - G.ring);
        }
    }
    for (int d = 32; d; d >>= 1) {
        hx ^= (unsigned)__shfl_xor((int)hx, d);
        hy += (unsigned)__shfl_xor((int)hy, d);
    }
    if (lane == 0) {
        wavehash[2 * wave] = hx;
        wavehash[2 * wave + 1] = hy;
    }
    __syncthreads();
    if constexpr (HALO) {
        if (wait_south) peer_halo_wait(&opaque(K)->H.counters[2], K->H.expect_done[0]);
        if (wait_north) peer_halo_wait(&opaque(K)->H.counters[3], K->H.expect_done[1]);
    }
    const DevParams& P = *lp;
    bool have_list = false;
    int nwet = 0;
    if (use_static) {
        unsigned got_x = 0, got_y = 0;
#pragma unroll
        for (int w = 0; w < Geo::WAVES; ++w) {
            got_x ^= wavehash[2 * w];
            got_y += wavehash[2 * w + 1];
        }
        have_list = got_x == want_x && got_y == want_y;
        nwet = listed;
        if (sort_windows > 1 && nwet > 0)
            inv_window = 1.0f / (float)(((nwet + sort_windows * 64 - 1) / (sort_windows * 64)) * 64);
    }
    if (have_list && land && !keep_land) {
        LeanArgsPtr Kz = opaque(K);
#pragma unroll
        for (int n = 0; n < LAND_UNROLL; ++n)
            if (land & (1u << n)) {
                const int idx = range_begin + tid + n * BLOCK;
                const int jj = row_of(idx, wx, wx_rcp);
                const int i = idx - jj * wx - G.ring, j = jj - G.ring;
                lean_zero_cell<FUSE>(L, T_offset, G, Kz, cell_index(G, i, j), i, j);
            }
    }
    int begin = range_begin, end = range_end;
    for (;;) {
        if (!have_list) {
            for (int base = begin; base < end; base += BLOCK) {
                const int idx = base + tid;
                bool wet = false;
                if (idx < end) {
                    const int jj = row_of(idx, wx, wx_rcp);
                    const int i = idx - jj * wx - G.ring, j = jj - G.ring;
                    const size_t k = cell_index(G, i, j);
                    wet = cell_is_wet(P, mask, k);
                    if (!wet) lean_zero_cell<FUSE>(L, T_offset, G, opaque(K), k, i, j);
                }
                const unsigned long long m = __ballot(wet);
                int wave_base = 0;
                if (lane == 0 && m) wave_base = atomicAdd(&counters[2], __popcll(m));
                wave_base = __shfl(wave_base, 0);
                if (wet) {
                    const int p = wave_base + __popcll(m & ((1ull << lane) - 1ull));
                    if (p < CHUNK) list[p] = (unsigned)(idx - range_begin);
                }
            }
            __syncthreads();
            nwet = counters[2];
            if (nwet > CHUNK) {
                end = begin + CHUNK;
                __syncthreads();
                if (tid < 4) counters[tid] = 0;
                if constexpr (CERT) {
                    if (tid < 2 * AO_BINS) hist[tid] = -1;
                }
                __syncthreads();
                continue;
            }
        }
        auto store_result = [&](double* base, unsigned byte_off, double v) {
            if constexpr (FUSE) gstore_final(base, byte_off, v);
            else gstore(base, byte_off, v);
        };
        auto claim = [&]() {
            int st = 0;
            if (lane == 0) st = atomicAdd(&counters[0], 64);
            return __shfl(st, 0);
        };
        constexpr int QUEUE_CAP = 2 * AO_BINS;
        constexpr int QUEUE_CLOSED = 1 << 20;
        int* queue = hist;
        static_assert(Geo::CURSOR_OFFSET == Geo::HIST_OFFSET + AO_BINS * 4, "the exact-path queue spans the histogram and the cursors");
        bool straggling = false;
        int limit = nwet;
        auto position_of = [&](int st) -> int {
            const int qq = min(st + lane, limit - 1);
            if constexpr (CERT) return straggling ? queue[qq] : qq;
            return qq;
        };
        auto coords_of = [&](int st, int& ci, int& cj) -> size_t {
            const int idx = range_begin + (int)(list[position_of(st)] & LEAN_OFFSET_MASK);
            const int jj = row_of(idx, wx, wx_rcp);
            ci = idx - jj * wx - G.ring;
            cj = jj - G.ring;
            return cell_index(G, ci, cj);
        };
        auto cell_of = [&](int st) -> size_t {
            int ci, cj;
            return coords_of(st, ci, cj);
        };
        struct Raw {
            double ua, va, Ta, pa, qa, u0, u1, v0, v1, To, So;
        };
        auto request = [&](int st) {
            int ci, cj;
            const size_t k = coords_of(st, ci, cj);
            LeanArgsPtr Kb = opaque(K);
            const double* __restrict__ Ou = Kb->O.u;
            const double* __restrict__ Ov = Kb->O.v;
            const unsigned k8 = (unsigned)k * 8u;
            Raw r;
            r.u0 = gload(Ou, k8);
            r.u1 = gload(Ou, k8 + 8u);
            r.v0 = gload(Ov, k8);
            r.v1 = gload(Ov, k8 + (unsigned)G.sj * 8u);
            r.To = gload(Kb->O.T, k8);
            r.So = gload(Kb->O.S, k8);
            r.ua = gload(Kb->E.u, k8);
            r.va = gload(Kb->E.v, k8);
            r.Ta = gload(Kb->E.T, k8);
            r.pa = gload(Kb->E.p, k8);
            r.qa = gload(Kb->E.q, k8);
            return r;
        };
        int start = claim();
        Raw raw{};
        if (start < nwet) raw = request(start);
        for (;;) {
            if constexpr (CERT) {
                if (!straggling && start >= nwet) {
                    int filled = 0;
                    if (lane == 0) filled = atomicAdd(&counters[1], QUEUE_CLOSED);
                    filled = __shfl(filled, 0);
                    if (filled <= 0 || filled >= QUEUE_CLOSED) break;
                    limit = min(filled, QUEUE_CAP);
                    for (int e = lane; e < limit; e += 64)
                        while (__hip_atomic_load(&queue[e], __ATOMIC_ACQUIRE, __HIP_MEMORY_SCOPE_WORKGROUP) < 0) __builtin_amdgcn_s_sleep(1);
                    straggling = true;
                    start = 0;
                    raw = request(start);
                }
            }
            if (start >= limit) break;
            const int q = start + lane;
            const bool in_range = q < limit;
            double Mp_now = 0.0;
            const double raw_So = raw.So;
            if constexpr (CERT) {
                if (!straggling) Mp_now = gload(opaque(K)->E.Mp, (unsigned)cell_of(start) * 8u);
            }
            const LeanCell c = lean_prologue(P, L.kappa, tab, raw.ua, raw.va, raw.Ta, raw.pa, raw.qa, 0.5 * (raw.u0 + raw.u1),
                                             0.5 * (raw.v0 + raw.v1), raw.To, raw.So);
            if (in_range) store_result(opaque(K)->F.Ts, (unsigned)cell_of(start) * 8u, c.Ts - T_offset);
            CertNetSalt net_salt;
            if constexpr (CERT) {
                net_salt.Mp = (float)Mp_now;
                net_salt.floor_v = CERT_JS_FLOOR * __builtin_amdgcn_rcpf((float)raw_So * (float)P.rho_f_inv);
            }
            Scales s;
            bool finish = in_range;
            if constexpr (CERT) {
                bool exact = in_range;
                if (!straggling) {
                    const LoopParams Lc = kread(&opaque(K)->L);
                    s = mo_iterate_certified<COARE>(Lc, c, tab, in_range, exact, net_salt);
                    const unsigned long long m = __builtin_amdgcn_ballot_w64(exact);
                    const bool in_place = ((volatile int*)counters)[1] == 0 && ((volatile int*)counters)[0] >= nwet;
                    if (m && !in_place) {
                        int slot = 0;
                        if (lane == 0) slot = atomicAdd(&counters[1], __popcll(m));
                        slot = __shfl(slot, 0) + __popcll(m & ((1ull << lane) - 1ull));
                        if (exact && slot < QUEUE_CAP) {
                            __hip_atomic_store(&queue[slot], q, __ATOMIC_RELEASE, __HIP_MEMORY_SCOPE_WORKGROUP);
                            exact = false;
                            finish = false;
                        }
                    }
                }
                if (__builtin_amdgcn_ballot_w64(exact) != 0ull) {
                    const LoopParams Le = kread(&opaque(K)->L);
                    const Scales e = mo_iterate_lean<COARE, false>(Le, c, tab, exact);
                    if (exact) {
                        s = e;
                        s.it |= CERT_EXACT_FLAG;
                    }
                }
            } else {
                if constexpr (LINE) s = mo_iterate_lean_line<COARE>(L, c, tab, in_range);
                else s = mo_iterate_lean<COARE>(L, c, tab, in_range);
            }
            if (finish) {
                LeanArgsPtr Ke = opaque(K);
                const size_t k = cell_of(start);
                const CellFluxes R = lean_epilogue(c, T_offset, s);
                const FluxOut F = kread(&Ke->F);
                const unsigned k8 = (unsigned)k * 8u;
                store_result(F.Qc, k8, R.Qc);
                store_result(F.Qv, k8, R.Qv);
                store_result(F.Fv, k8, R.Fv);
                gstore(F.tx, k8, R.rho_tau_x);
                gstore(F.ty, k8, R.rho_tau_y);
                if (F.ustar) gstore_final(F.ustar, k8, R.ustar);
                if (F.tstar) gstore_final(F.tstar, k8, R.tstar);
                if (F.qstar) gstore_final(F.qstar, k8, R.qstar);
                if (F.iters) gstore_i32(F.iters, (unsigned)k * 4u, R.iterations);
                if constexpr (FUSE) {
                    const int idx = range_begin + (int)(list[position_of(start)] & LEAN_OFFSET_MASK);
                    const int jj = row_of(idx, wx, wx_rcp);
                    const int ci = idx - jj * wx - G.ring, cj = jj - G.ring;
                    if (ci >= 0 && ci < G.nx && cj >= 0 && cj < G.ny) {
// ... 67 lines not shown
```

climaocean.jl_amd/csrc/coflux_solver_lean.hip:

```cpp
#include <hip/hip_runtime.h>

#include <cstring>

#include "coflux_lean_kernel.hpp"

namespace coflux {

template <bool COARE, bool FUSE, bool TAIL = false, bool CERT = false>
__global__ __launch_bounds__(AO_BLOCK, LEAN_WAVES) void ao_lean_kernel(LeanArgs unused_by_name) {
    ao_lean_body<COARE, FUSE, TAIL, CERT>((LeanArgsPtr)__builtin_amdgcn_kernarg_segment_ptr(), (int)blockIdx.x);
}

template <bool COARE>
__global__ __launch_bounds__(AO_BLOCK, LEAN_WAVES) void ao_lean_halo_kernel(LeanArgs unused_by_name) {
    ao_lean_body<COARE, true, true, false, false, true>((LeanArgsPtr)__builtin_amdgcn_kernarg_segment_ptr(), (int)blockIdx.x);
}

__global__ __launch_bounds__(256) void lean_list_build_kernel(const uint32_t* __restrict__ wet_pos, const int* __restrict__ begins, int stride,
                                                              uint32_t* __restrict__ sorted, int* __restrict__ info) {
    __shared__ unsigned sx[4], sy[4];
    __shared__ int sn[4];
    const int chunk = blockIdx.x, lane = threadIdx.x & 63, wave = threadIdx.x >> 6;
    const int begin = begins[chunk];
    unsigned hx = 0, hy = 0;
    int n = 0;
    for (int e = threadIdx.x; e < stride; e += 256) {
        const uint32_t idx = wet_pos[(size_t)chunk * stride + e];
        const bool listed = idx != 0xffffffffu;
        sorted[(size_t)chunk * stride + e] = listed ? idx - (uint32_t)begin : LEAN_OFFSET_MASK;
        if (listed) {
            hx ^= lean_mix(idx);
            hy += lean_sum(idx);
            ++n;
        }
    }
    for (int d = 32; d; d >>= 1) {
        hx ^= (unsigned)__shfl_xor((int)hx, d);
        hy += (unsigned)__shfl_xor((int)hy, d);
        n += __shfl_xor(n, d);
    }
    if (lane == 0) {
        sx[wave] = hx;
        sy[wave] = hy;
        sn[wave] = n;
    }
    __syncthreads();
    if (threadIdx.x == 0) {
        info[chunk * 4] = sn[0] + sn[1] + sn[2] + sn[3];
        info[chunk * 4 + 1] = (int)(sx[0] ^ sx[1] ^ sx[2] ^ sx[3]);
        info[chunk * 4 + 2] = (int)(sy[0] + sy[1] + sy[2] + sy[3]);
        info[chunk * 4 + 3] = 0;
    }
}

hipError_t build_lean_lists(hipStream_t st, int nchunks, const uint32_t* d_wet_pos, const int* d_begins, uint32_t* d_sorted, int* d_info) {
    hipLaunchKernelGGL(lean_list_build_kernel, dim3(nchunks), dim3(256), 0, st, d_wet_pos, d_begins, AO_CHUNK, d_sorted, d_info);
    return hipGetLastError();
}

bool lean_certified_applies(const LaunchCfg& L, const LoopParams& C) {
    return L.certified && C.specialization == SOLVER_OCEAN_LEAN && !C.fixed && L.lean_hints == 0 &&
           C.cert_max_evals > 2 && C.tol >= 1e-9 && C.maxiter >= 40;
}

bool lean_halo_rides(const LaunchCfg& L, const LoopParams& C) {
    return C.specialization == SOLVER_OCEAN_LEAN && L.solver == CF_SOLVER_TABLES && !lean_certified_applies(L, C);
}

bool lean_line_applies(const LaunchCfg& L, const LoopParams& C, bool coare) {
    if (L.latency_layout == 0 || C.specialization != SOLVER_OCEAN_LEAN || C.beta_gust == 0.0) return false;
    if (lean_certified_applies(L, C)) return false;
    return L.latency_layout == 2 || (coare && L.cu_count > 0 && L.n_chunks <= 2 * L.cu_count);
}

static hipError_t fill_lean_args(const LaunchCfg& L, const DevParams& P, const LoopParams& C, const GridDesc& G, const cf_ocean_surface* o,
                                 const cf_exchange_fields* e, const cf_interface_fluxes* f, const cf_sea_ice_fields* ice,
                                 const cf_net_ocean_fluxes* net, const double* land, LeanArgs& A) {
    if (!L.d_chunk_begins || L.n_chunks <= 0 || !L.d_lean_info) return hipErrorInvalidValue;
    A.L = C;
    A.G = G;
    A.O = make_ocean(o);
    A.E = make_exchange(e);
    A.F = make_fluxes(f);
    A.g_tab = L.d_tables;
    A.g_params = L.d_params;
    A.sorted = L.d_wet_pos ? L.d_lean_sorted : nullptr;
    A.info = L.d_lean_info;
    A.chunk_begins = L.d_chunk_begins;
    A.z_surface = P.z_surface;
    A.mask_kind = P.mask_kind;
    A.T_offset = P.T_offset;
    A.wx_reciprocal = row_reciprocal(G.nx + 2 * G.ring);
    A.sort_enabled = L.lean_hints;
    A.keep_land = L.keep_land;
    if (net) {
        A.I = make_ice_in(ice, land);
        A.N = make_net_out(net);
    }
    return hipSuccess;
}

hipError_t make_ocean_rider(const LaunchCfg& L, const DevParams& P, const LoopParams& C, const GridDesc& G, const cf_ocean_surface* o,
                            const cf_exchange_fields* e, const cf_interface_fluxes* f, const cf_sea_ice_fields* ice,
                            const cf_net_ocean_fluxes* net, const double* land, OceanRider* out) {
    static_assert(sizeof(LeanArgs) <= sizeof(out->args), "OceanRider::args holds a LeanArgs");
    if (!out || !net) return hipErrorInvalidValue;
    LeanArgs A{};
    if (hipError_t err = fill_lean_args(L, P, C, G, o, e, f, ice, net, land, A)) return err;
    memcpy(out->args, &A, sizeof(A));
    out->n_chunks = L.n_chunks;
    out->coare = P.similarity_form == CF_SIMILARITY_COARE_LOGARITHMIC;
    out->valid = true;
    return hipSuccess;
}

hipError_t launch_ao_fluxes_lean(hipStream_t st, const LaunchCfg& L, const DevParams& P, const LoopParams& C, const GridDesc& G,
                                 const cf_ocean_surface* o, const cf_exchange_fields* e, const cf_interface_fluxes* f,
                                 const cf_sea_ice_fields* ice, const cf_net_ocean_fluxes* net, const double* land,
                                 const cf_atmos_source* next_src, const cf_interp_weights* w, const cf_exchange_fields* next_out,
                                 int tail_rows, int tail_blocks, const HaloRider* halo) {
    LeanArgs A{};
    if (hipError_t err = fill_lean_args(L, P, C, G, o, e, f, ice, net, land, A)) return err;
    const bool coare = P.similarity_form == CF_SIMILARITY_COARE_LOGARITHMIC;
    const bool cert = lean_certified_applies(L, C);
    const bool tail = next_out != nullptr;
    int blocks = L.n_chunks;
    if (tail) {
        if (!net || !next_src || !w || L.interp_cap <= 0 || tail_blocks <= 0) return hipErrorInvalidValue;
        const size_t tile_lds = (size_t)IT_WAVES * CF_JRA55_NVARS * L.interp_cap * sizeof(double);
        if (tile_lds > (size_t)LeanGeom<AO_BLOCK>::LDS_BYTES) return hipErrorInvalidValue;
        A.S = make_source(next_src);
        A.Wt = make_weights(w);
        A.E_next = make_exchange(next_out);
        A.n_chunks = L.n_chunks;
        A.tail_blocks = tail_blocks;
        A.tail_rows = tail_rows;
        A.tail_cap = L.interp_cap;
        A.tail_pos = L.n_chunks;
        blocks += tail_blocks;
    }
    const bool riders = halo != nullptr && halo->blocks > 0;
    if (riders) {
        if (!tail || !lean_halo_rides(L, C) || halo->F.n < 1 || halo->blocks != 2 * halo->F.n) return hipErrorInvalidValue;
        A.H = *halo;
        blocks += halo->blocks;
    }
    if (lean_line_applies(L, C, coare)) return launch_ao_lean_line(st, coare, net != nullptr, tail, riders, blocks, A);
    if (riders) {
        if (coare) hipLaunchKernelGGL((ao_lean_halo_kernel<true>), dim3(blocks), dim3(AO_BLOCK), LeanGeom<AO_BLOCK>::LDS_BYTES, st, A);
        else hipLaunchKernelGGL((ao_lean_halo_kernel<false>), dim3(blocks), dim3(AO_BLOCK), LeanGeom<AO_BLOCK>::LDS_BYTES, st, A);
        return hipGetLastError();
    }
#define CF_LEAN_LAUNCH(COARE_, FUSE_, TAIL_, CERT_) \
    hipLaunchKernelGGL((ao_lean_kernel<COARE_, FUSE_, TAIL_, CERT_>), dim3(blocks), dim3(AO_BLOCK), LeanGeom<AO_BLOCK>::LDS_BYTES, st, A)
#define CF_LEAN_PICK(FUSE_, TAIL_)                                                       \
    do {                                                                                 \
        if (cert) {                                                                      \
            if (coare) CF_LEAN_LAUNCH(true, FUSE_, TAIL_, true); else CF_LEAN_LAUNCH(false, FUSE_, TAIL_, true);   \
        } else {                                                                         \
            if (coare) CF_LEAN_LAUNCH(true, FUSE_, TAIL_, false); else CF_LEAN_LAUNCH(false, FUSE_, TAIL_, false); \
        }                                                                                \
    } while (0)
    if (tail) CF_LEAN_PICK(true, true);
    else if (net) CF_LEAN_PICK(true, false);
    else CF_LEAN_PICK(false, false);
#undef CF_LEAN_PICK
#undef CF_LEAN_LAUNCH
    return hipGetLastError();
}

}
```

include/coflux.h:

```cpp
#ifndef COFLUX_H
#define COFLUX_H

#include <stddef.h>
#include <stdint.h>

#ifdef __cplusplus
extern "C" {
#endif

#define CF_ABI_VERSION 5

#define CF_OK 0
#define CF_ERR_INVALID (-1)
#define CF_ERR_HIP (-2)
#define CF_ERR_NODEVICE (-3)
#define CF_ERR_COMM (-4)

typedef struct cf_ctx cf_ctx;

typedef struct cf_grid {
    int32_t nx, ny;
    int32_t hx, hy;
    int32_t ring;
    int32_t reserved;
// ... 130 lines not shown
typedef struct cf_exchange_fields {
    double* u;
    double* v;
    double* T;
    double* p;
    double* q;
    double* Qs;
    double* Ql;
    double* Mp;
} cf_exchange_fields;

typedef struct cf_interface_fluxes {
    double* sensible_heat;
    double* latent_heat;
    double* water_vapor;
    double* x_momentum;
    double* y_momentum;
    double* temperature;
    double* friction_velocity;
    double* temperature_scale;
    double* humidity_scale;
    int32_t* iterations;
} cf_interface_fluxes;

typedef struct cf_sea_ice_fields {
    const double* concentration;
    const double* interface_heat;
    const double* salt_flux;
    const double* x_stress;
    const double* y_stress;
} cf_sea_ice_fields;

typedef struct cf_net_ocean_fluxes {
    double* u;
    double* v;
    double* T;
    double* S;
    double* shortwave_surface_flux;
    double* upwelling_longwave;
    double* downwelling_longwave;
    double* downwelling_shortwave;
} cf_net_ocean_fluxes;

#define CF_JRA55_TAS 0
#define CF_JRA55_HUSS 1
#define CF_JRA55_PSL 2
#define CF_JRA55_UAS 3
#define CF_JRA55_VAS 4
#define CF_JRA55_RLDS 5
#define CF_JRA55_RSDS 6
#define CF_JRA55_PRRA 7
#define CF_JRA55_PRSN 8
#define CF_JRA55_NVARS 9

typedef struct cf_atmos_source {
    const float* data[CF_JRA55_NVARS];
    int32_t ns_x, ns_y;
    int32_t n_levels;
    int32_t level1, level2;
    double time_fraction;
} cf_atmos_source;

typedef struct cf_interp_weights {
    int32_t separable;
    int32_t reserved;
    const double* fi;
    const double* fj;
    const double* cos_rot;
    const double* sin_rot;
    const double* latitude;
} cf_interp_weights;

int cf_version(void);
const char* cf_build_stamp(void);
int cf_create(cf_ctx** out, int device, const cf_grid* grid, const cf_flux_params* params);
int cf_destroy(cf_ctx* ctx);
const char* cf_last_error(const cf_ctx* ctx);
int cf_set_flux_params(cf_ctx* ctx, const cf_flux_params* params);
#define CF_STREAM_LEGACY ((void*)1)
int cf_set_stream(cf_ctx* ctx, void* hip_stream);

#define CF_OPT_SOLVER 0
#define CF_OPT_LAND_ZEROS 2
#define CF_OPT_INTERP_TILE_CAP 1
#define CF_OPT_TRIP_HINTS 3
#define CF_OPT_AO_CHUNK 4
#define CF_OPT_FUSED_NET 6
#define CF_OPT_MERGED_PREFETCH 9
#define CF_OPT_ICE_ORBIT_SHORTCUT 7
#define CF_OPT_SOLVER_PATH 10
#define CF_SOLVER_PATH_EXACT 0
#define CF_SOLVER_PATH_CERTIFIED 1
#define CF_CERTIFIED_EXACT_FLAG 0x100
#define CF_OPT_CERTIFIED_BUDGET 11
#define CF_OPT_ICE_FREE_CELLS 12
#define CF_ICE_FREE_ITERATE 0
#define CF_OPT_LATENCY_LAYOUT 13
#define CF_ICE_FREE_ZERO 1
#define CF_OPT_HALO_IN_SOLVER_LAUNCH 14
#define CF_OPT_INTERP_TILE_ROWS 15
#define CF_SOLVER_TABLES 0
#define CF_SOLVER_LIBM 1
int cf_set_option(cf_ctx* ctx, int option, int value);
int cf_solver_iteration_path(cf_ctx* ctx, int* path);
int cf_solver_latency_layout(cf_ctx* ctx, int* layout);
int cf_debug_eval(cf_ctx* ctx, int function, int n, const double* d_x, double* d_y);
int cf_debug_chunk_plan(long long total_cost, int cu_count, int forced_wet_per_chunk, int* out, int capacity);
int cf_debug_chunk_table(cf_ctx* ctx, int* begins, int* wet_counts, int capacity, int* n_chunks, int* lists_valid);
int cf_debug_land_zero_launches(cf_ctx* ctx, int* launches);
int cf_debug_interp_grid(cf_ctx* ctx, int* rows, int* blocks);
int cf_sync(cf_ctx* ctx);

void* cf_device_alloc(cf_ctx* ctx, size_t bytes);
int cf_device_free(cf_ctx* ctx, void* d_ptr);
int cf_h2d(cf_ctx* ctx, void* d_dst, const void* h_src, size_t bytes);
int cf_d2h(cf_ctx* ctx, void* h_dst, const void* d_src, size_t bytes);


int cf_interpolate_atmosphere_state(cf_ctx* ctx, const cf_atmos_source* src,
                                    const cf_interp_weights* w, const cf_exchange_fields* out);

int cf_compute_atmosphere_ocean_fluxes(cf_ctx* ctx, const cf_ocean_surface* ocean,
                                       const cf_exchange_fields* atmos,
                                       const cf_interface_fluxes* out);

int cf_compute_net_ocean_fluxes(cf_ctx* ctx, const cf_ocean_surface* ocean,
                                const cf_exchange_fields* atmos,
                                const cf_interface_fluxes* fluxes,
                                const cf_sea_ice_fields* ice ,
                                const cf_interp_weights* w ,
                                const cf_net_ocean_fluxes* out);

int cf_update_state(cf_ctx* ctx, const cf_atmos_source* src, const cf_interp_weights* w,
                    const cf_ocean_surface* ocean, const cf_exchange_fields* atmos,
                    const cf_interface_fluxes* fluxes, const cf_sea_ice_fields* ice,
                    const cf_net_ocean_fluxes* net);

typedef struct cf_window cf_window;
int cf_window_create(cf_ctx* ctx, int32_t ns_x, int32_t ns_y, int32_t n_slots, cf_window** out);
int cf_window_destroy(cf_window* w);
float* cf_window_host_buffer(cf_window* w, int32_t slot, int32_t variable);
int cf_window_wait_slot(cf_window* w, int32_t slot);
int cf_window_commit(cf_window* w, int32_t slot, int64_t time_index);
int cf_window_upload(cf_window* w, int64_t time_index, const float* const* host_vars);
int cf_window_find(cf_window* w, int64_t time_index);
int cf_window_source(cf_window* w, int64_t n1, int64_t n2, double time_fraction, cf_atmos_source* out);

#define CF_SKIN_EXPLICIT 0
#define CF_SKIN_SEMI_IMPLICIT 1
#define CF_SKIN_LINEARISED 2
typedef struct cf_sea_ice_params {
    int32_t struct_size;
    int32_t skin_temperature_scheme;
    double conductivity;
    double consolidation_thickness;
    double maximum_temperature_change;
    double ice_salinity;
    double liquidus_slope;
    double freshwater_melting_temperature;
    double albedo;
    double emissivity;
    double temperature_offset;
} cf_sea_ice_params;

int cf_default_sea_ice_params(cf_sea_ice_params* p);

typedef struct cf_sea_ice_state {
    const double* concentration;
    const double* thickness;
    const double* top_temperature;
    const double* u;
    const double* v;
    const double* albedo;
    const double* snow_thickness;
} cf_sea_ice_state;

typedef struct cf_sea_ice_albedo_params {
    int32_t struct_size;
    int32_t reserved;
    double ice_visible, ice_near_infrared;
    double snow_visible, snow_near_infrared;
    double ocean_albedo;
    double reference_thickness;
    double melt_temperature_range;
    double ice_melt_change;
    double snow_melt_change_visible;
    double snow_melt_change_near_infrared;
    double snow_patch_thickness;
    double visible_fraction;
    double melting_temperature;
} cf_sea_ice_albedo_params;
int cf_default_sea_ice_albedo_params(cf_sea_ice_albedo_params* p);
// ... 436 lines not shown
```

Measured before the change: 10.24 billion cells/s.

## Trust verified wet-cell lists within a step loop and preload first cell

Within a cf_time_steps loop, once a launch has verified the per-chunk wet lists against the mask hash, later launches with the same key skip the mask scan and hash reduction. A device-side stale flag lets the kernel fall back to verification if a list ever fails its check. When lists are trusted, each wave also issues the global loads for its first listed cell before the table and list LDS-DMA staging, to hide that latency behind the staging. This adds cross-step state and a device flag read per block, and relies on the mask not changing inside a loop without the generation key changing.

Result: no change. 10.28 billion cells/s (median of 5 runs) (+0.4%).

```diff
diff --git a/climaocean.jl_amd/coflux/abi.py b/climaocean.jl_amd/coflux/abi.py
--- a/climaocean.jl_amd/coflux/abi.py
+++ b/climaocean.jl_amd/coflux/abi.py
@@ -26,6 +26,8 @@
 OPT_SOLVER_PATH, OPT_CERTIFIED_BUDGET, OPT_ICE_FREE_CELLS, OPT_LATENCY_LAYOUT, OPT_HALO_IN_SOLVER_LAUNCH = 10, 11, 12, 13, 14
 OPT_LAND_ZEROS = 2
 LAND_ZEROS_EVERY_LAUNCH, LAND_ZEROS_AUTO, LAND_ZEROS_NEVER = 0, 1, 2
+OPT_TRUSTED_LISTS = 5
+TRUSTED_LISTS_OFF, TRUSTED_LISTS_AUTO = 0, 1
 ICE_FREE_ITERATE, ICE_FREE_ZERO = 0, 1
 PIPELINE_WITHIN_CALL, PIPELINE_CONTINUING = 1, 2
 AVERAGE_MAX_FIELDS = 16
@@ -328,7 +330,7 @@
     "cf_interpolate_land_freshwater", "cf_set_land_freshwater", "cf_materialize_salinity_restoring",
     "cf_window_create", "cf_window_destroy", "cf_window_host_buffer", "cf_window_wait_slot", "cf_window_commit",
     "cf_window_upload", "cf_window_find", "cf_window_source",
-    "cf_ensure_chunk_table", "cf_debug_chunk_table", "cf_debug_interp_grid", "cf_debug_land_zero_launches", "cf_solver_path", "cf_solver_iteration_path", "cf_solver_latency_layout", "cf_comm_count", "cf_build_stamp", "cf_discard_prefetched_atmosphere_state",
+    "cf_ensure_chunk_table", "cf_debug_chunk_table", "cf_debug_interp_grid", "cf_debug_land_zero_launches", "cf_debug_trusted_lists", "cf_solver_path", "cf_solver_iteration_path", "cf_solver_latency_layout", "cf_comm_count", "cf_build_stamp", "cf_discard_prefetched_atmosphere_state",
     "cf_debug_prefetch_stats",
     "cf_average_create", "cf_average_destroy", "cf_average_reset", "cf_average_collect", "cf_average_weight", "cf_attach_average",
     "cf_average_create_derived", "cf_average_create_budget", "cf_attach_average_slot",
@@ -463,6 +465,7 @@
     lib.cf_debug_chunk_table.argtypes = [vp, C.POINTER(C.c_int), C.POINTER(C.c_int), C.c_int, C.POINTER(C.c_int), C.POINTER(C.c_int)]
     lib.cf_debug_interp_grid.argtypes = [vp, C.POINTER(C.c_int), C.POINTER(C.c_int)]
     lib.cf_debug_land_zero_launches.argtypes = [vp, C.POINTER(C.c_int)]
+    lib.cf_debug_trusted_lists.argtypes = [vp, C.POINTER(C.c_int), C.POINTER(C.c_int)]
     lib.cf_solver_path.argtypes = [vp, C.POINTER(C.c_int), C.POINTER(C.c_int)]
     lib.cf_default_sea_ice_albedo_params.argtypes = [C.POINTER(SeaIceAlbedoParams)]
     lib.cf_set_sea_ice_albedo.argtypes = [vp, C.POINTER(SeaIceAlbedoParams)]
diff --git a/climaocean.jl_amd/coflux/runtime.py b/climaocean.jl_amd/coflux/runtime.py
--- a/climaocean.jl_amd/coflux/runtime.py
+++ b/climaocean.jl_amd/coflux/runtime.py
@@ -297,6 +297,11 @@
         n = C.c_int()
         self._check(self.lib.cf_debug_land_zero_launches(self._h, C.byref(n)), "cf_debug_land_zero_launches")
         return n.value
+
+    def debug_trusted_lists(self):
+        n, stale = C.c_int(), C.c_int()
+        self._check(self.lib.cf_debug_trusted_lists(self._h, C.byref(n), C.byref(stale)), "cf_debug_trusted_lists")
+        return n.value, stale.value
 
     def solver_path(self):
         lean, fused = C.c_int(), C.c_int()
diff --git a/climaocean.jl_amd/csrc/coflux_abi.cpp b/climaocean.jl_amd/csrc/coflux_abi.cpp
--- a/climaocean.jl_amd/csrc/coflux_abi.cpp
+++ b/climaocean.jl_amd/csrc/coflux_abi.cpp
@@ -235,6 +235,10 @@
         }
     }
     if (n <= 0 || n + 1 > chunk_table_capacity(ncells)) return fail(ctx, CF_ERR_HIP, "chunk table of %d entries is invalid", n);
+    if (!ctx->d_lists_stale) HIP_TRY(ctx, ctx->d_lists_stale.create(sizeof(int)));
+    HIP_TRY(ctx, hipMemsetAsync(ctx->d_lists_stale.get(), 0, sizeof(int), ctx->stream));
+    ctx->launch.d_lists_stale = ctx->d_lists_stale.get();
+    ++ctx->chunk_generation;
     ctx->chunk_mask = key;
     ctx->chunk_mask_kind = d.mask_kind;
     ctx->chunk_z_surface = d.z_surface;
@@ -563,6 +567,10 @@
                 return fail(ctx, CF_ERR_INVALID, "CF_OPT_LAND_ZEROS = 2 is an experiment value: start the process with COFLUX_EXPERIMENTS=1");
             ctx->land_zeros = value;
             return CF_OK;
+        case CF_OPT_TRUSTED_LISTS:
+            if (value < 0 || value > 1) return fail(ctx, CF_ERR_INVALID, "trusted lists %d: 0 (every launch verifies its wet lists) or 1 (automatic: the first step of a cf_time_steps call)", value);
+            ctx->trusted_lists = value;
+            return CF_OK;
         default: return fail(ctx, CF_ERR_INVALID, "unknown option %d", option);
     }
 }
@@ -748,6 +756,18 @@
     const bool fixed_trips = ctx->fast.specialization == SOLVER_LY && ctx->launch.solver == CF_SOLVER_TABLES;
     return (ctx->fused_net == 1 || (ctx->fused_net == 2 && (lean || fixed_trips))) && ctx->launch.solver == CF_SOLVER_TABLES &&
            ctx->dev.albedo_kind == CF_ALBEDO_CONSTANT;
+}
+
+int cf_debug_trusted_lists(cf_ctx* ctx, int* trusted_launches, int* stale) {
+    if (!ctx || !trusted_launches || !stale) return fail(ctx, CF_ERR_INVALID, "cf_debug_trusted_lists: bad arguments");
+    *trusted_launches = ctx->step_loop.trusted_launches;
+    *stale = 0;
+    if (ctx->d_lists_stale) {
+        HIP_TRY(ctx, hipSetDevice(ctx->device));
+        HIP_TRY(ctx, hipMemcpyAsync(stale, ctx->d_lists_stale.get(), sizeof(int), hipMemcpyDeviceToHost, ctx->stream));
+        HIP_TRY(ctx, hipStreamSynchronize(ctx->stream));
+    }
+    return CF_OK;
 }
 
 int cf_solver_iteration_path(cf_ctx* ctx, int* path) {
@@ -865,11 +885,18 @@
             CHECK(cf_peer_halo_launch_now(ctx, &halo_request.F, halo_request.rows));
         }
     }
-    const unsigned way = 1u | (fuse ? 2u : 0u) | (ride ? 4u : 0u) | ((unsigned)ctx->fast.specialization << 3);
+    StepKey key;
+    key.way = 1u | (fuse ? 2u : 0u) | (ride ? 4u : 0u) | ((unsigned)ctx->fast.specialization << 3);
+    key.mask = ctx->chunk_mask;
+    key.mask_kind = ctx->chunk_mask_kind;
+    key.generation = ctx->chunk_generation;
     const bool knows = ctx->launch.solver == CF_SOLVER_TABLES;
-    const bool keep_land = knows && (ctx->land_zeros == 2 || (ctx->land_zeros == 1 && ctx->step_loop.open && ctx->step_loop.last_way == way));
+    const bool has_lists = knows && ctx->fast.specialization == SOLVER_OCEAN_LEAN && ctx->launch.d_wet_pos != nullptr;
+    const StepDecision decision = step_decide(ctx->step_loop, ctx->land_zeros, ctx->trusted_lists, knows, has_lists, key);
+    const bool keep_land = decision.keep_land;
     LaunchCfg L = ctx->launch;
     L.keep_land = keep_land ? 1 : 0;
+    L.trust_lists = decision.trust_lists ? 1 : 0;
     if (ride) {
         HIP_TRY(ctx, make_ocean_rider(L, ctx->dev, ctx->fast, ctx->grid, ocean, atmos, fluxes, ice, net, ctx->d_land_freshwater,
                                       ocean_rider));
@@ -894,7 +921,6 @@
     } else
     HIP_TRY(ctx, launch_ao_fluxes(ctx->stream, L, ctx->dev, ctx->fast, ctx->grid, ocean, atmos, fluxes,
                                   fuse ? ice : nullptr, fuse ? net : nullptr, ctx->d_land_freshwater));
-    if (ctx->step_loop.open && !keep_land) ++ctx->step_loop.zero_launches;
     const bool merge = fuse && !hold_tail_work && ctx->merged_prefetch == 1 && next && interp_tile_fits(ctx, 65536);
     if (ctx->merged_prefetch == 0) {
         const AheadLedger::Work behind_solver = ctx->ahead.leave_aux();
@@ -920,7 +946,7 @@
         HIP_TRY(ctx, launch_interpolate(ctx->stream, ctx->launch, ctx->grid, &next->src, &next->w, &next->out));
         ctx->ahead.leave_main(next, AheadLedger::OWN);
     }
-    if (ctx->step_loop.open) ctx->step_loop.last_way = way;
+    step_record(ctx->step_loop, key, decision);
     return CF_OK;
 }
 
diff --git a/climaocean.jl_amd/csrc/coflux_ctx.hpp b/climaocean.jl_amd/csrc/coflux_ctx.hpp
--- a/climaocean.jl_amd/csrc/coflux_ctx.hpp
+++ b/climaocean.jl_amd/csrc/coflux_ctx.hpp
@@ -26,6 +26,7 @@
 #include "coflux_kernels.h"
 #include "coflux_owned.hpp"
 #include "coflux_request_ahead.hpp"
+#include "coflux_step_scope.hpp"
 #include "coflux_tables.h"
 
 using namespace coflux;
@@ -34,6 +35,10 @@
 #define CF_LAND_ZEROS_DEFAULT 1
 #endif
 static_assert(CF_LAND_ZEROS_DEFAULT == 0 || CF_LAND_ZEROS_DEFAULT == 1, "the experiment value is not a default");
+#ifndef CF_TRUSTED_LISTS_DEFAULT
+#define CF_TRUSTED_LISTS_DEFAULT 1
+#endif
+static_assert(CF_TRUSTED_LISTS_DEFAULT == 0 || CF_TRUSTED_LISTS_DEFAULT == 1, "off or automatic");
 
 struct RcclApi {
     void* handle = nullptr;
@@ -116,6 +121,8 @@
     double chunk_z_surface = 0.0;
     int chunk_wet = 0;
     bool chunk_valid = false;
+    uint64_t chunk_generation = 0;
+    cf::DeviceBuffer<int> d_lists_stale;
     cf::DeviceBuffer<double> d_reduce;
     bool ice_ready = false;
     cf_flux_params ice_params{};
@@ -163,11 +170,8 @@
         int rows = 0;
     } halo_request;
     int land_zeros = CF_LAND_ZEROS_DEFAULT;
-    struct StepLoop {
-        bool open = false;
-        unsigned last_way = 0;
-        int zero_launches = 0;
-    } step_loop;
+    int trusted_lists = CF_TRUSTED_LISTS_DEFAULT;
+    StepLoop step_loop;
     ncclComm_t comm = nullptr;
     int rank = 0, nranks = 1;
     std::vector<cf::Event> prof_events;
@@ -181,14 +185,8 @@
 
 struct LandZeroScope {
     cf_ctx* ctx;
-    explicit LandZeroScope(cf_ctx* c) : ctx(c) {
-        ctx->step_loop = cf_ctx::StepLoop{};
-        ctx->step_loop.open = true;
-    }
-    ~LandZeroScope() {
-        ctx->step_loop.open = false;
-        ctx->step_loop.last_way = 0;
-    }
+    explicit LandZeroScope(cf_ctx* c) : ctx(c) { step_loop_open(ctx->step_loop); }
+    ~LandZeroScope() { step_loop_close(ctx->step_loop); }
     LandZeroScope(const LandZeroScope&) = delete;
     LandZeroScope& operator=(const LandZeroScope&) = delete;
 };
diff --git a/climaocean.jl_amd/csrc/coflux_kernels.h b/climaocean.jl_amd/csrc/coflux_kernels.h
--- a/climaocean.jl_amd/csrc/coflux_kernels.h
+++ b/climaocean.jl_amd/csrc/coflux_kernels.h
@@ -38,6 +38,8 @@
     int certified;
     int latency_layout;
     int keep_land;
+    int trust_lists;
+    int* d_lists_stale;
 };
 
 bool lean_line_applies(const LaunchCfg& L, const LoopParams& C, bool coare);
diff --git a/climaocean.jl_amd/csrc/coflux_lean_kernel.hpp b/climaocean.jl_amd/csrc/coflux_lean_kernel.hpp
--- a/climaocean.jl_amd/csrc/coflux_lean_kernel.hpp
+++ b/climaocean.jl_amd/csrc/coflux_lean_kernel.hpp
@@ -10,6 +10,10 @@
 namespace coflux {
 
 constexpr int LEAN_WAVES = 3;
+
+#ifndef CF_TRUSTED_LISTS_DEAL_FIRST
+#define CF_TRUSTED_LISTS_DEAL_FIRST 1
+#endif
 
 struct LeanArgs {
     LoopParams L;
@@ -37,6 +41,8 @@
     long long tail_pos;
     HaloRider H;
     long long keep_land;
+    long long trust_lists;
+    int* lists_stale;
 };
 typedef const LeanArgs __attribute__((address_space(4)))* LeanArgsPtr;
 
@@ -150,36 +156,29 @@
     const int wx = G.nx + 2 * G.ring;
     const unsigned wx_rcp = (unsigned)K->wx_reciprocal;
     const bool use_static = K->sorted != nullptr;
-    static_assert(sizeof(DevParams) % 16 == 0 && sizeof(DevParams) <= 1024, "the parameter block is one LDS-DMA piece");
-    if (tid < (int)(sizeof(DevParams) / 16))
-        __builtin_amdgcn_global_load_lds((const __attribute__((address_space(1))) void*)(reinterpret_cast<const char*>(g_params) + lane * 16),
-                                         (__attribute__((address_space(3))) void*)(smem + Geo::PARAMS_OFFSET), 16, 0, 0);
-    static_assert(TABLE_BYTES % 1024 == 0, "the table stage copies whole 1 KB pieces");
-    {
-        const char* gb = reinterpret_cast<const char*>(g_tab);
-        constexpr int PIECES = TABLE_BYTES / 1024, WAVES = Geo::WAVES;
-#pragma unroll
-        for (int r = 0; r < (PIECES + WAVES - 1) / WAVES; ++r) {
-            const int c = wave + r * WAVES;
-            if (c < PIECES)
-                __builtin_amdgcn_global_load_lds((const __attribute__((address_space(1))) void*)(gb + c * 1024 + lane * 16),
-                                                 (__attribute__((address_space(3))) void*)(smem + c * 1024), 16, 0, 0);
-        }
-    }
-    if (use_static) {
-        const char* gl = reinterpret_cast<const char*>(K->sorted + (size_t)chunk * CHUNK);
-        constexpr int PIECES = CHUNK * 4 / 1024, WAVES = Geo::WAVES;
-#pragma unroll
-        for (int r = 0; r < (PIECES + WAVES - 1) / WAVES; ++r) {
-            const int c = wave + r * WAVES;
-            if (c < PIECES)
-                __builtin_amdgcn_global_load_lds((const __attribute__((address_space(1))) void*)(gl + c * 1024 + lane * 16),
-                                                 (__attribute__((address_space(3))) void*)(smem + LEAN_LIST_OFFSET + c * 1024), 16, 0, 0);
-        }
-    }
-    constexpr int LAND_UNROLL = 8;
     typedef const __attribute__((address_space(1))) unsigned* GlobalWords;
-    unsigned raw_lo[LAND_UNROLL], raw_hi[LAND_UNROLL], raw_shift = 0;
+    struct Raw {
+        double ua, va, Ta, pa, qa, u0, u1, v0, v1, To, So;
+    };
+    auto request_cell = [&](size_t k) {
+        LeanArgsPtr Kb = opaque(K);
+        const double* __restrict__ Ou = Kb->O.u;
+        const double* __restrict__ Ov = Kb->O.v;
+        const unsigned k8 = (unsigned)k * 8u;
+        Raw r;
+        r.u0 = gload(Ou, k8);
+        r.u1 = gload(Ou, k8 + 8u);
+        r.v0 = gload(Ov, k8);
+        r.v1 = gload(Ov, k8 + (unsigned)G.sj * 8u);
+        r.To = gload(Kb->O.T, k8);
+        r.So = gload(Kb->O.S, k8);
+        r.ua = gload(Kb->E.u, k8);
+        r.va = gload(Kb->E.v, k8);
+        r.Ta = gload(Kb->E.T, k8);
+        r.pa = gload(Kb->E.p, k8);
+        r.qa = gload(Kb->E.q, k8);
+        return r;
+    };
     const __attribute__((address_space(4))) int* cb = (const __attribute__((address_space(4))) int*)K->chunk_begins;
     const int range_begin = cb[chunk], range_end = cb[chunk + 1];
     int listed = 0;
@@ -194,6 +193,8 @@
     const double z_surface = K->z_surface;
     const double T_offset = K->T_offset;
     const bool keep_land = K->keep_land != 0;
+    const bool trust_handed = (int)(K->trust_lists != 0) & (int)keep_land & (int)use_static;
+    bool trusted = false;
     const bool sorting = !CERT && use_static && K->sort_enabled != 0;
     const int sort_windows = (int)K->sort_enabled;
     float inv_window = 0.f;
@@ -203,7 +204,60 @@
         const int bpw = AO_BINS / sort_windows, lo = bpw >= 16 ? 5 : 8;
         return w * bpw + (bpw - 1 - min(max(trips - lo, 0), bpw - 1));
     };
+    constexpr bool PRELOAD = !LINE && CF_TRUSTED_LISTS_DEAL_FIRST != 0;
+    bool preloaded = false;
+    int start = 0;
+    Raw raw{};
+    if (trust_handed) {
+        unsigned first_entry = 0;
+        if constexpr (PRELOAD) first_entry = *(GlobalWords)(K->sorted + (size_t)chunk * CHUNK + tid);
+        trusted = ((const __attribute__((address_space(4))) int*)K->lists_stale)[0] == 0;
+        if constexpr (PRELOAD) asm volatile("" : "+v"(first_entry));
+        if constexpr (PRELOAD) {
+            const int first_mine = 64 * __builtin_amdgcn_readfirstlane(wave);
+            if (trusted && !(wait_south || wait_north) && first_mine < listed) {
+                const int last_lane = min(listed - 1 - first_mine, 63);
+                const unsigned last_entry = (unsigned)__builtin_amdgcn_readlane((int)first_entry, last_lane);
+                const unsigned entry = lane <= last_lane ? first_entry : last_entry;
+                const int idx = range_begin + (int)(entry & LEAN_OFFSET_MASK);
+                const int jj = row_of(idx, wx, wx_rcp);
+                raw = request_cell(cell_index(G, idx - jj * wx - G.ring, jj - G.ring));
+                start = first_mine;
+                preloaded = true;
+            }
+        }
+    }
+    const bool deal_first = PRELOAD && trusted && !(wait_south || wait_north);
+    static_assert(sizeof(DevParams) % 16 == 0 && sizeof(DevParams) <= 1024, "the parameter block is one LDS-DMA piece");
+    if (tid < (int)(sizeof(DevParams) / 16))
+        __builtin_amdgcn_global_load_lds((const __attribute__((address_space(1))) void*)(reinterpret_cast<const char*>(g_params) + lane * 16),
+                                         (__attribute__((address_space(3))) void*)(smem + Geo::PARAMS_OFFSET), 16, 0, 0);
+    static_assert(TABLE_BYTES % 1024 == 0, "the table stage copies whole 1 KB pieces");
     {
+        const char* gb = reinterpret_cast<const char*>(g_tab);
+        constexpr int PIECES = TABLE_BYTES / 1024, WAVES = Geo::WAVES;
+#pragma unroll
+        for (int r = 0; r < (PIECES + WAVES - 1) / WAVES; ++r) {
+            const int c = wave + r * WAVES;
+            if (c < PIECES)
+                __builtin_amdgcn_global_load_lds((const __attribute__((address_space(1))) void*)(gb + c * 1024 + lane * 16),
+                                                 (__attribute__((address_space(3))) void*)(smem + c * 1024), 16, 0, 0);
+        }
+    }
+    if (use_static) {
+        const char* gl = reinterpret_cast<const char*>(K->sorted + (size_t)chunk * CHUNK);
+        constexpr int PIECES = CHUNK * 4 / 1024, WAVES = Geo::WAVES;
+#pragma unroll
+        for (int r = 0; r < (PIECES + WAVES - 1) / WAVES; ++r) {
+            const int c = wave + r * WAVES;
+            if (c < PIECES)
+                __builtin_amdgcn_global_load_lds((const __attribute__((address_space(1))) void*)(gl + c * 1024 + lane * 16),
+                                                 (__attribute__((address_space(3))) void*)(smem + LEAN_LIST_OFFSET + c * 1024), 16, 0, 0);
+        }
+    }
+    constexpr int LAND_UNROLL = 8;
+    unsigned raw_lo[LAND_UNROLL], raw_hi[LAND_UNROLL], raw_shift = 0;
+    if (!trusted) {
         const unsigned long long mbase = mask_kind == CF_MASK_NONE ? (unsigned long long)g_tab : (unsigned long long)mask;
         const unsigned stride = mask_kind == CF_MASK_NONE ? 0u : (mask_kind == CF_MASK_U8 ? 1u : 8u);
         const unsigned hi_step = mask_kind == CF_MASK_BOTTOM_HEIGHT ? 4u : 0u;
@@ -217,49 +271,51 @@
             raw_hi[n] = *(GlobalWords)((a & ~3ull) + hi_step);
         }
     }
-    if (tid < 4) counters[tid] = 0;
+    if (tid < 4) counters[tid] = tid == 0 && deal_first ? 64 * Geo::WAVES : 0;
     if (tid < AO_BINS) hist[tid] = 0;
     if constexpr (CERT) {
         if (tid < 2 * AO_BINS) hist[tid] = -1;
     }
     __builtin_amdgcn_s_waitcnt(0x0f70);
-#pragma unroll
-    for (int n = 0; n < LAND_UNROLL; ++n) asm volatile("" : "+v"(raw_lo[n]), "+v"(raw_hi[n]));
     unsigned hx = 0, hy = 0, land = 0;
-#pragma unroll
-    for (int n = 0; n < LAND_UNROLL; ++n) {
-        const int idx = range_begin + tid + n * BLOCK;
-        const bool w = mask_kind == CF_MASK_NONE ? true
-                       : mask_kind == CF_MASK_U8 ? ((raw_lo[n] >> (8 * ((raw_shift >> (2 * n)) & 3u))) & 0xffu) != 0
-                                                 : !(z_surface <= __hiloint2double((int)raw_hi[n], (int)raw_lo[n]));
-        if (idx < range_end) {
+    if (!trusted) {
+#pragma unroll
+        for (int n = 0; n < LAND_UNROLL; ++n) asm volatile("" : "+v"(raw_lo[n]), "+v"(raw_hi[n]));
+#pragma unroll
+        for (int n = 0; n < LAND_UNROLL; ++n) {
+            const int idx = range_begin + tid + n * BLOCK;
+            const bool w = mask_kind == CF_MASK_NONE ? true
+                           : mask_kind == CF_MASK_U8 ? ((raw_lo[n] >> (8 * ((raw_shift >> (2 * n)) & 3u))) & 0xffu) != 0
+                                                     : !(z_surface <= __hiloint2double((int)raw_hi[n], (int)raw_lo[n]));
+            if (idx < range_end) {
+                if (w) {
+                    hx ^= lean_mix((unsigned)idx);
+                    hy += lean_sum((unsigned)idx);
+                } else {
+                    land |= 1u << n;
+                }
+            }
+        }
+        for (int idx = range_begin + tid + LAND_UNROLL * BLOCK; idx < range_end; idx += BLOCK) {
+            const int jj = row_of(idx, wx, wx_rcp);
+            const size_t k = cell_index(G, idx - jj * wx - G.ring, jj - G.ring);
+            const bool w = mask_kind == CF_MASK_NONE ? true
+                           : mask_kind == CF_MASK_U8 ? ((const uint8_t*)mask)[k] != 0 : !(z_surface <= ((const double*)mask)[k]);
             if (w) {
                 hx ^= lean_mix((unsigned)idx);
                 hy += lean_sum((unsigned)idx);
-            } else {
-                land |= 1u << n;
-            }
-        }
-    }
-    for (int idx = range_begin + tid + LAND_UNROLL * BLOCK; idx < range_end; idx += BLOCK) {
-        const int jj = row_of(idx, wx, wx_rcp);
-        const size_t k = cell_index(G, idx - jj * wx - G.ring, jj - G.ring);
-        const bool w = mask_kind == CF_MASK_NONE ? true
-                       : mask_kind == CF_MASK_U8 ? ((const uint8_t*)mask)[k] != 0 : !(z_surface <= ((const double*)mask)[k]);
-        if (w) {
-            hx ^= lean_mix((unsigned)idx);
-            hy += lean_sum((unsigned)idx);
-        } else if (!keep_land) {
-            lean_zero_cell<FUSE>(L, T_offset, G, opaque(K), k, idx - jj * wx - G.ring, jj - G.ring);
-        }
-    }
-    for (int d = 32; d; d >>= 1) {
-        hx ^= (unsigned)__shfl_xor((int)hx, d);
-        hy += (unsigned)__shfl_xor((int)hy, d);
-    }
-    if (lane == 0) {
-        wavehash[2 * wave] = hx;
-        wavehash[2 * wave + 1] = hy;
+            } else if (!keep_land) {
+                lean_zero_cell<FUSE>(L, T_offset, G, opaque(K), k, idx - jj * wx - G.ring, jj - G.ring);
+            }
+        }
+        for (int d = 32; d; d >>= 1) {
+            hx ^= (unsigned)__shfl_xor((int)hx, d);
+            hy += (unsigned)__shfl_xor((int)hy, d);
+        }
+        if (lane == 0) {
+            wavehash[2 * wave] = hx;
+            wavehash[2 * wave + 1] = hy;
+        }
     }
     __syncthreads();
     if constexpr (HALO) {
@@ -276,7 +332,7 @@
             got_x ^= wavehash[2 * w];
             got_y += wavehash[2 * w + 1];
         }
-        have_list = got_x == want_x && got_y == want_y;
+        have_list = trusted || (got_x == want_x && got_y == want_y);
         nwet = listed;
         if (sort_windows > 1 && nwet > 0)
             inv_window = 1.0f / (float)(((nwet + sort_windows * 64 - 1) / (sort_windows * 64)) * 64);
@@ -292,6 +348,7 @@
                 lean_zero_cell<FUSE>(L, T_offset, G, Kz, cell_index(G, i, j), i, j);
             }
     }
+    if (!have_list && tid == 0) gstore_i32(opaque(K)->lists_stale, 0u, 1);
     int begin = range_begin, end = range_end;
     for (;;) {
         if (!have_list) {
@@ -358,33 +415,12 @@
             int ci, cj;
             return coords_of(st, ci, cj);
         };
-        struct Raw {
-            double ua, va, Ta, pa, qa, u0, u1, v0, v1, To, So;
-        };
-        auto request = [&](int st) {
-            int ci, cj;
-            const size_t k = coords_of(st, ci, cj);
-            LeanArgsPtr Kb = opaque(K);
-            const double* __restrict__ Ou = Kb->O.u;
-            const double* __restrict__ Ov = Kb->O.v;
-            const unsigned k8 = (unsigned)k * 8u;
-            Raw r;
-            r.u0 = gload(Ou, k8);
-            r.u1 = gload(Ou, k8 + 8u);
-            r.v0 = gload(Ov, k8);
-            r.v1 = gload(Ov, k8 + (unsigned)G.sj * 8u);
-            r.To = gload(Kb->O.T, k8);
-            r.So = gload(Kb->O.S, k8);
-            r.ua = gload(Kb->E.u, k8);
-            r.va = gload(Kb->E.v, k8);
-            r.Ta = gload(Kb->E.T, k8);
-            r.pa = gload(Kb->E.p, k8);
-            r.qa = gload(Kb->E.q, k8);
-            return r;
-        };
-        int start = claim();
-        Raw raw{};
-        if (start < nwet) raw = request(start);
+        auto request = [&](int st) { return request_cell(cell_of(st)); };
+        if (!preloaded) {
+            start = claim();
+            if (start < nwet) raw = request(start);
+        }
+        preloaded = false;
         for (;;) {
             if constexpr (CERT) {
                 if (!straggling && start >= nwet) {
diff --git a/climaocean.jl_amd/csrc/coflux_solver_lean.hip b/climaocean.jl_amd/csrc/coflux_solver_lean.hip
--- a/climaocean.jl_amd/csrc/coflux_solver_lean.hip
+++ b/climaocean.jl_amd/csrc/coflux_solver_lean.hip
@@ -76,7 +76,7 @@
 static hipError_t fill_lean_args(const LaunchCfg& L, const DevParams& P, const LoopParams& C, const GridDesc& G, const cf_ocean_surface* o,
                                  const cf_exchange_fields* e, const cf_interface_fluxes* f, const cf_sea_ice_fields* ice,
                                  const cf_net_ocean_fluxes* net, const double* land, LeanArgs& A) {
-    if (!L.d_chunk_begins || L.n_chunks <= 0 || !L.d_lean_info) return hipErrorInvalidValue;
+    if (!L.d_chunk_begins || L.n_chunks <= 0 || !L.d_lean_info || !L.d_lists_stale) return hipErrorInvalidValue;
     A.L = C;
     A.G = G;
     A.O = make_ocean(o);
@@ -93,6 +93,8 @@
     A.wx_reciprocal = row_reciprocal(G.nx + 2 * G.ring);
     A.sort_enabled = L.lean_hints;
     A.keep_land = L.keep_land;
+    A.trust_lists = L.keep_land && L.trust_lists;
+    A.lists_stale = L.d_lists_stale;
     if (net) {
         A.I = make_ice_in(ice, land);
         A.N = make_net_out(net);
diff --git a/climaocean.jl_amd/csrc/coflux_step_scope.hpp b/climaocean.jl_amd/csrc/coflux_step_scope.hpp
--- /dev/null
+++ b/climaocean.jl_amd/csrc/coflux_step_scope.hpp
@@ -0,0 +1,59 @@
+#pragma once
+#include <cstdint>
+
+namespace coflux {
+
+struct StepKey {
+    unsigned way = 0;
+    const void* mask = nullptr;
+    int mask_kind = -1;
+    uint64_t generation = 0;
+    bool same_lists(const StepKey& o) const { return way == o.way && mask == o.mask && mask_kind == o.mask_kind && generation == o.generation; }
+};
+
+struct StepDecision {
+    bool keep_land = false;
+    bool trust_lists = false;
+};
+
+struct StepLoop {
+    bool open = false;
+    unsigned last_way = 0;
+    bool verified = false;
+    StepKey verified_key;
+    int zero_launches = 0;
+    int trusted_launches = 0;
+};
+
+inline StepDecision step_decide(const StepLoop& loop, int land_zeros, int trusted_lists, bool knows, bool has_lists, const StepKey& key) {
+    StepDecision d;
+    d.keep_land = knows && (land_zeros == 2 || (land_zeros == 1 && loop.open && loop.last_way == key.way));
+    d.trust_lists = d.keep_land && has_lists && trusted_lists == 1 && land_zeros == 1 && loop.open && loop.verified &&
+                    loop.verified_key.same_lists(key);
+    return d;
+}
+
+inline void step_record(StepLoop& loop, const StepKey& key, const StepDecision& d) {
+    if (!loop.open) return;
+    if (!d.keep_land) ++loop.zero_launches;
+    if (d.trust_lists) {
+        ++loop.trusted_launches;
+    } else {
+        loop.verified = true;
+        loop.verified_key = key;
+    }
+    loop.last_way = key.way;
+}
+
+inline void step_loop_open(StepLoop& loop) {
+    loop = StepLoop{};
+    loop.open = true;
+}
+inline void step_loop_close(StepLoop& loop) {
+    loop.open = false;
+    loop.last_way = 0;
+    loop.verified = false;
+    loop.verified_key = StepKey{};
+}
+
+}
diff --git a/include/coflux.h b/include/coflux.h
--- a/include/coflux.h
+++ b/include/coflux.h
@@ -236,6 +236,7 @@
 
 #define CF_OPT_SOLVER 0
 #define CF_OPT_LAND_ZEROS 2
+#define CF_OPT_TRUSTED_LISTS 5
 #define CF_OPT_INTERP_TILE_CAP 1
 #define CF_OPT_TRIP_HINTS 3
 #define CF_OPT_AO_CHUNK 4
@@ -262,6 +263,7 @@
 int cf_debug_chunk_plan(long long total_cost, int cu_count, int forced_wet_per_chunk, int* out, int capacity);
 int cf_debug_chunk_table(cf_ctx* ctx, int* begins, int* wet_counts, int capacity, int* n_chunks, int* lists_valid);
 int cf_debug_land_zero_launches(cf_ctx* ctx, int* launches);
+int cf_debug_trusted_lists(cf_ctx* ctx, int* trusted_launches, int* stale);
 int cf_debug_interp_grid(cf_ctx* ctx, int* rows, int* blocks);
 int cf_sync(cf_ctx* ctx);
 
```
